# index-tts/index-tts

Measured on AMD Instinct MI355X. Metric: audio-seconds/sec (RTF) IndexTTS-2.5, 64-utt batch @1/2/4/8 MI355X, higher is better.
Workload: dtype bf16 (GPT GEMM operands / KV cache; f32 accumulate, residual stream, norms: the reference's own GPU mode) + fp32x3 (flow matching: f32 activations / weights / accumulation, GEMM and attention products on the bf16 matrix pipe with every f32 operand carried exactly as three bf16 planes = 24 significan

## Files before the change

include/indextts_hip.h:

```cpp
#ifndef INDEXTTS_HIP_H
#define INDEXTTS_HIP_H

#include <stddef.h>
#include <stdint.h>

#ifdef __cplusplus
extern "C" {
#endif

#define ITTS_ABI_VERSION 13

int itts_abi_version(void);
const char* itts_last_error(void);
int itts_device_count(void);

int itts_set_option(const char* name, int value);
int itts_get_option(const char* name, int* value);
int itts_reset_options(void);
int itts_option_count(void);
const char* itts_option_name(int index);
const char* itts_option_doc(int index);
int itts_option_default(int index);


// ... 108 lines not shown
void itts_gpt_destroy(itts_gpt* h);
size_t itts_gpt_workspace_bytes(const itts_gpt* h, int nseq, int S, int Tmax);

int itts_gpt_generate(itts_gpt* h, const float* prefix_embeds, const int32_t* pad_lens, int nseq, int S,
                      const itts_gen_params* params, const int32_t* penalty_ids, int n_penalty_ids,
                      const double* uniforms, int64_t* codes_out, int32_t* n_steps_out, void* workspace,
                      size_t workspace_bytes, int use_graph, void* stream);
int itts_gpt_generate_chunk(itts_gpt* h, const float* prefix_embeds, const int32_t* pad_lens, int nseq, int S,
                            const itts_gen_params* params, const int32_t* penalty_ids, int n_penalty_ids,
                            const double* uniforms, int64_t* codes_out, int32_t step_limit, int32_t* n_steps_out,
                            void* workspace, size_t workspace_bytes, int use_graph, void* stream);
size_t itts_gpt_admit_workspace_bytes(const itts_gpt* h, int n_new, int S_new);
int itts_gpt_admit_rows(itts_gpt* h, const float* prefix_embeds, const int32_t* pad_lens, const int32_t* slots, int n_new, int S_new,
                        const int32_t* row_limits_new, const itts_gen_params* params, const int32_t* penalty_ids, int n_penalty_ids,
                        const double* uniforms, int64_t* codes_out, void* workspace, size_t workspace_bytes, void* admit_workspace,
                        size_t admit_bytes, void* stream);
size_t itts_gpt_beam_workspace_bytes(const itts_gpt* h, int n_utts, int num_beams, int S, int Tmax);
int itts_gpt_generate_beam(itts_gpt* h, const float* prefix_embeds, const int32_t* pad_lens, int n_utts, int num_beams,
                           int S, const itts_gen_params* params, const int32_t* penalty_ids, int n_penalty_ids,
                           const double* uniforms, int32_t* hist_tok_out, int32_t* hist_par_out, float* beam_scores_out,
                           float* hyps_out, int32_t* n_hyps_out, uint8_t* done_out, int32_t* n_steps_out,
                           void* workspace, size_t workspace_bytes, int use_graph, void* stream);
int itts_gpt_generate_beam_chunk(itts_gpt* h, const float* prefix_embeds, const int32_t* pad_lens, int n_utts, int num_beams, int S,
                                 const itts_gen_params* params, const int32_t* penalty_ids, int n_penalty_ids, const int32_t* group_caps,
                                 int32_t* hist_tok_out, int32_t* hist_par_out, float* beam_scores_out, float* hyps_out, int32_t* n_hyps_out,
                                 uint8_t* done_out, int32_t step_limit, int32_t* n_steps_out, void* workspace, size_t workspace_bytes,
                                 int use_graph, void* stream);
size_t itts_gpt_admit_beam_workspace_bytes(const itts_gpt* h, int n_new, int S_new);
int itts_gpt_admit_beam_groups(itts_gpt* h, const float* prefix_embeds, const int32_t* pad_lens, const int32_t* slots, int n_new, int S_new,
                               const int32_t* group_caps_new, const itts_gen_params* params, const int32_t* penalty_ids, int n_penalty_ids,
                               void* workspace, size_t workspace_bytes, void* admit_workspace, size_t admit_bytes, void* stream);
int itts_gpt_last_timing(const itts_gpt* h, float* prefill_ms, float* decode_ms, int32_t* steps);
int itts_gpt_graph_stats(const itts_gpt* h, int32_t* captures, int32_t* hits);
int itts_gpt_set_compaction(itts_gpt* h, int enable, int granularity);
int itts_gpt_set_chunk_return(itts_gpt* h, int finished_rows);
int itts_gpt_set_row_limits(itts_gpt* h, const int32_t* limits, int n);
typedef struct {
    int32_t  do_sample, top_k, min_tokens_to_keep;
    float    top_p, temperature, repetition_penalty, typical_mass;
    int32_t  stream;
    uint64_t seed;
} itts_row_sampling;
int itts_gpt_set_row_sampling(itts_gpt* h, const itts_row_sampling* table, int n);
typedef struct {
    int32_t  do_sample, top_k, min_tokens_to_keep;
    float    top_p, temperature, repetition_penalty, typical_mass, length_penalty;
    int32_t  stream;
    uint64_t seed;
} itts_group_sampling;
int itts_gpt_set_group_sampling(itts_gpt* h, const itts_group_sampling* table, int n_groups);
typedef struct {
    int32_t  min_new_tokens;
    int32_t  min_length;
    int32_t  no_repeat_ngram_size;
    int32_t  decay_start;
    float    min_p;
    float    epsilon_cutoff;
    float    eta_cutoff;
    int32_t  n_suppress, n_begin_suppress, n_decay;
    const int32_t* suppress_ids;
    const int32_t* begin_suppress_ids;
    const float*   decay_table;
} itts_logits_filters;
int itts_gpt_set_logits_filters(itts_gpt* h, const itts_logits_filters* f);
int itts_gpt_compaction_stats(const itts_gpt* h, int64_t* row_steps, int32_t* compactions);

int itts_gpt_forward_latent(itts_gpt* h, const float* x, int nseq, int S, float* out, void* workspace,
                            size_t workspace_bytes, void* stream);

typedef struct itts_gpt_latent itts_gpt_latent;
size_t itts_gpt_latent_workspace_bytes(const itts_gpt* h, int nseq, int max_prefix, int max_codes, int max_append);
int itts_gpt_latent_open(itts_gpt* h, const float* prefix_x, const int32_t* prefix_lens, int nseq, int max_prefix, int max_codes,
                         int max_append, void* workspace, size_t workspace_bytes, void* stream, itts_gpt_latent** session);
int itts_gpt_latent_append(itts_gpt_latent* session, const int64_t* codes, int n, float* out, void* stream);
int itts_gpt_latent_appended(const itts_gpt_latent* session);
int itts_gpt_latent_close(itts_gpt_latent* session);

int itts_gemm_tile_occupancy(int precision, int32_t* blocks_per_cu);
const char* itts_gemm_last_path(void);
int itts_gemm_path_count(void);
const char* itts_gemm_path_name(int index);
int itts_gemm_forward(const void* A, const void* Wp, const float* bias, float* out, int M, int N, int K, int precision,
                      int prefill_tiles, int gelu, void* stream);
int itts_layernorm_forward(const float* x, const float* gamma, const float* beta, const float* gamma2,
                           const float* beta2, float* out, int rows, int D, float eps, void* stream);
const char* itts_attention_last_path(void);
int itts_attention_path_count(void);
const char* itts_attention_path_name(int index);
int itts_gpt_attention_forward(const float* q, const void* kcache, const void* vcache, void* out, const int32_t* pos_ptr, const int32_t* pad,
                               const int32_t* pos_shift, const int32_t* seq_map, const int32_t* row_map, const int32_t* row_map_alt,
                               const int32_t* step_ptr, int nseq, int heads, int nq, int Tmax, int seq_mul, int precision, void* stream);
int itts_gemm_ln_forward(const float* x, const float* partial, const float* bias_prev, const float* ln_gamma, const float* ln_beta, float eps,
                         const void* Wp, const float* bias, float* out, float* x_out, int M, int N, int K, void* stream);

typedef struct {
    int32_t hidden_dim, num_heads, depth;
    int32_t in_channels;
    int32_t wavenet_hidden, wavenet_layers, wavenet_kernel, wavenet_dilation_rate;
    int32_t precision;
    float norm_eps;
} itts_s2mel_config;

typedef struct itts_s2mel itts_s2mel;

int itts_s2mel_create(const itts_s2mel_config* cfg, itts_s2mel** out);
int itts_s2mel_device(const itts_s2mel* h);
int itts_s2mel_load_tensor(itts_s2mel* h, const char* name, const float* host_data, const int64_t* shape, int ndim);
int itts_s2mel_finalize(itts_s2mel* h);
void itts_s2mel_destroy(itts_s2mel* h);
size_t itts_s2mel_workspace_bytes(const itts_s2mel* h, int n_tok, int n_seq, int t_max);
int itts_s2mel_mods_per_step(const itts_s2mel* h);

int itts_s2mel_estimator(itts_s2mel* h, const float* x, const float* const_in, const float* mods, const float* rope,
                         const int32_t* tok_seq, const int32_t* tok_t, const int32_t* seq_start, const int32_t* seq_T,
                         const int32_t* seq_len, int n_seq, int n_tok, int t_max, float* d_out, void* workspace,
                         size_t workspace_bytes, void* stream);
int itts_s2mel_solve(itts_s2mel* h, float* x_state, const float* const_in, const float* mods, const float* rope,
                     const int32_t* tok_seq, const int32_t* tok_t, const int32_t* seq_start, const int32_t* seq_T,
                     const int32_t* seq_len, const int32_t* prompt_len, int n_seq, int n_tok, int t_max, int n_branch, int n_steps,
                     const float* t_span, float cfg_rate, void* workspace, size_t workspace_bytes, void* stream);

int itts_s2mel_set_profiling(itts_s2mel* h, int enable);
int itts_s2mel_profile_read(itts_s2mel* h, double* ms, double* launches, double* flops);

int itts_s2mel_set_trace(itts_s2mel* h, void* dev_u64, int capacity);
int itts_s2mel_trace_count(const itts_s2mel* h);
int itts_s2mel_trace_wanted(const itts_s2mel* h);
const char* itts_s2mel_trace_label(const itts_s2mel* h, int index);
int itts_s2mel_set_capture(itts_s2mel* h, void* dev_buf, size_t bytes, const char* label_prefix);
long long itts_s2mel_capture_offset(const itts_s2mel* h, int index, size_t* bytes);

int itts_s2mel_set_tail(itts_s2mel* h, const int32_t* tok_seq, const int32_t* tok_t, const int32_t* seq_start, const int32_t* seq_T,
                        const int32_t* seq_len, const int32_t* tail_src, const int32_t* tail_base, int n_seq, int n_tail, int t_max);

int itts_s2mel_noise_forward(float* x_rows, const int32_t* tok_seq, const int32_t* tok_t, const int32_t* prompt_len,
                             const uint64_t* seq_seed, const uint64_t* seq_key, const float* seq_temperature,
                             int n_seq, int n_rows, int channels, void* stream);

size_t itts_s2mel_attention_scratch_bytes(int n_tok, int n_seq, int heads, int t_max, int precision);
int itts_s2mel_attention_forward(const float* qkv, const float* rope, const int32_t* tok_seq, const int32_t* tok_t,
                                 const int32_t* seq_start, const int32_t* seq_T, const int32_t* seq_len, int n_seq, int n_tok,
                                 int t_max, int heads, int precision, void* out, void* scratch, size_t scratch_bytes, void* stream);

int itts_vq_project_forward(const int64_t* codes, const float* codebook, const float* w, const float* bias, float* out, int n,
                            int n_codes, int cd, int H, void* stream);
int itts_vq_search_forward(const float* h, const float* w_in, const float* b_in, const float* cb_norm, const float* cb_sq, int64_t* idx,
                           int n, int H, int n_codes, int cd, void* stream);
int itts_tok_gather_conv_forward(const float* x, float* col, const int32_t* tok_seq, const int32_t* tok_t, const int32_t* src_start,
                                 const int32_t* src_T, const int32_t* dst_T, int n_dst, int C, int k, void* stream);
int itts_tok_dwconv_forward(const float* x, const float* w, const float* b, float* y, const int32_t* tok_seq, const int32_t* tok_t,
                            const int32_t* seq_T, int n, int C, int k, void* stream);
int itts_tok_gelu_forward(float* x, size_t n, void* stream);
int itts_tok_scale_residual_forward(float* x, const float* y, const float* gamma, int n, int C, void* stream);
int itts_tok_groupnorm_mish_forward(float* x, const float* gamma, const float* beta, const int32_t* seq_start, const int32_t* seq_T,
                                    int n_seq, int C, float eps, void* stream);

int itts_attention_forward(const float* q, const float* k, const float* v, float* out, const int32_t* kstart, const int32_t* klen,
                           int n_q, int heads, int dq, int dv, float scale, void* stream);
int itts_attention_relkey_forward(const float* q, const float* k, const float* v, float* out, const int32_t* kstart, const int32_t* klen,
                                  const int32_t* qpos, const float* dist_emb, int left, int right, int n_q, int heads, int dq, int dv,
                                  float scale, void* stream);
int itts_tok_dwconv_causal_forward(const float* x, const float* w, const float* b, float* y, const int32_t* tok_seq, const int32_t* tok_t,
                                   const int32_t* seq_T, int n, int C, int k, void* stream);
int itts_tok_glu_forward(const float* x, float* out, int n, int C, int mode, void* stream);
int itts_tok_act_forward(float* x, size_t n, int mode, void* stream);
int itts_tok_l2norm_forward(float* x, const float* gamma, int n, int C, float scale, void* stream);
// ... 35 lines not shown
```

indextts_amd/_lib.py:

```python
import ctypes as C
import os

HERE = os.path.dirname(os.path.abspath(__file__))
LIB_PATH = os.path.join(HERE, "csrc", "libindextts_hip.so")

c_f32p = C.POINTER(C.c_float)
c_i32p = C.POINTER(C.c_int32)
c_i64p = C.POINTER(C.c_int64)
vp = C.c_void_p


class BigVGANConfig(C.Structure):
    _fields_ = [
        ("in_channels", C.c_int32), ("upsample_initial_channel", C.c_int32), ("num_upsamples", C.c_int32),
        ("upsample_rates", C.c_int32 * 8), ("upsample_kernel_sizes", C.c_int32 * 8), ("num_kernels", C.c_int32),
        ("resblock_kernel_sizes", C.c_int32 * 4), ("num_dilations", C.c_int32),
        ("resblock_dilations", (C.c_int32 * 4) * 4), ("snake_logscale", C.c_int32), ("activation", C.c_int32),
        ("use_tanh_at_final", C.c_int32), ("use_bias_at_final", C.c_int32), ("cond_dim", C.c_int32),
        ("cond_in_each_up_layer", C.c_int32),
    ]


class S2MelConfig(C.Structure):
    _fields_ = [("hidden_dim", C.c_int32), ("num_heads", C.c_int32), ("depth", C.c_int32), ("in_channels", C.c_int32),
# ... 92 lines not shown
    "itts_packed_gemm_bytes": (C.c_size_t, [C.c_int, C.c_int, C.c_int]),
    "itts_pack_gemm_weight": (C.c_int, [vp, C.c_int, C.c_int, C.c_int, C.c_int, vp]),
    "itts_gpt_create": (C.c_int, [C.POINTER(GPTConfig), C.POINTER(vp)]),
    "itts_gpt_device": (C.c_int, [vp]),
    "itts_gpt_load_tensor": (C.c_int, [vp, C.c_char_p, vp, c_i64p, C.c_int]),
    "itts_gpt_finalize": (C.c_int, [vp]),
    "itts_gpt_destroy": (None, [vp]),
    "itts_gpt_workspace_bytes": (C.c_size_t, [vp, C.c_int, C.c_int, C.c_int]),
    "itts_gpt_generate": (C.c_int, [vp, vp, vp, C.c_int, C.c_int, C.POINTER(GenParams), c_i32p, C.c_int, vp, vp,
                                    C.POINTER(C.c_int32), vp, C.c_size_t, C.c_int, vp]),
    "itts_gpt_generate_chunk": (C.c_int, [vp, vp, vp, C.c_int, C.c_int, C.POINTER(GenParams), c_i32p, C.c_int, vp, vp, C.c_int32,
                                          C.POINTER(C.c_int32), vp, C.c_size_t, C.c_int, vp]),
    "itts_gpt_beam_workspace_bytes": (C.c_size_t, [vp, C.c_int, C.c_int, C.c_int, C.c_int]),
    "itts_gpt_generate_beam": (C.c_int, [vp, vp, vp, C.c_int, C.c_int, C.c_int, C.POINTER(GenParams), c_i32p, C.c_int, vp,
                                         vp, vp, vp, vp, vp, vp, C.POINTER(C.c_int32), vp, C.c_size_t, C.c_int, vp]),
    "itts_gpt_admit_workspace_bytes": (C.c_size_t, [vp, C.c_int, C.c_int]),
    "itts_gpt_admit_rows": (C.c_int, [vp, vp, vp, vp, C.c_int, C.c_int, vp, vp, vp, C.c_int, vp, vp, vp, C.c_size_t, vp, C.c_size_t, vp]),
    "itts_gpt_generate_beam_chunk": (C.c_int, [vp, vp, vp, C.c_int, C.c_int, C.c_int, C.POINTER(GenParams), c_i32p, C.c_int, c_i32p,
                                               vp, vp, vp, vp, vp, vp, C.c_int32, C.POINTER(C.c_int32), vp, C.c_size_t, C.c_int, vp]),
    "itts_gpt_admit_beam_workspace_bytes": (C.c_size_t, [vp, C.c_int, C.c_int]),
    "itts_gpt_admit_beam_groups": (C.c_int, [vp, vp, vp, c_i32p, C.c_int, C.c_int, c_i32p, C.POINTER(GenParams), c_i32p, C.c_int,
                                             vp, C.c_size_t, vp, C.c_size_t, vp]),
    "itts_gpt_last_timing": (C.c_int, [vp, C.POINTER(C.c_float), C.POINTER(C.c_float), C.POINTER(C.c_int32)]),
    "itts_gpt_graph_stats": (C.c_int, [vp, C.POINTER(C.c_int32), C.POINTER(C.c_int32)]),
    "itts_gpt_set_compaction": (C.c_int, [vp, C.c_int, C.c_int]),
    "itts_gpt_set_row_limits": (C.c_int, [vp, vp, C.c_int]),
    "itts_gpt_set_row_sampling": (C.c_int, [vp, vp, C.c_int]),
    "itts_gpt_set_group_sampling": (C.c_int, [vp, vp, C.c_int]),
    "itts_gpt_set_logits_filters": (C.c_int, [vp, C.POINTER(LogitsFilters)]),
    "itts_gpt_set_chunk_return": (C.c_int, [vp, C.c_int]),
    "itts_gpt_compaction_stats": (C.c_int, [vp, C.POINTER(C.c_int64), C.POINTER(C.c_int32)]),
    "itts_gpt_forward_latent": (C.c_int, [vp, vp, C.c_int, C.c_int, vp, vp, C.c_size_t, vp]),
    "itts_gpt_latent_workspace_bytes": (C.c_size_t, [vp, C.c_int, C.c_int, C.c_int, C.c_int]),
    "itts_gpt_latent_open": (C.c_int, [vp, vp, c_i32p, C.c_int, C.c_int, C.c_int, C.c_int, vp, C.c_size_t, vp, C.POINTER(vp)]),
    "itts_gpt_latent_append": (C.c_int, [vp, vp, C.c_int, vp, vp]),
    "itts_gpt_latent_appended": (C.c_int, [vp]),
    "itts_gpt_latent_close": (C.c_int, [vp]),
    "itts_gemm_tile_occupancy": (C.c_int, [C.c_int, C.POINTER(C.c_int32)]),
    "itts_s2mel_create": (C.c_int, [C.POINTER(S2MelConfig), C.POINTER(vp)]),
    "itts_s2mel_device": (C.c_int, [vp]),
    "itts_s2mel_load_tensor": (C.c_int, [vp, C.c_char_p, vp, c_i64p, C.c_int]),
    "itts_s2mel_set_tail": (C.c_int, [vp, vp, vp, vp, vp, vp, vp, vp, C.c_int, C.c_int, C.c_int]),
    "itts_s2mel_finalize": (C.c_int, [vp]),
    "itts_s2mel_destroy": (None, [vp]),
    "itts_s2mel_workspace_bytes": (C.c_size_t, [vp, C.c_int, C.c_int, C.c_int]),
    "itts_s2mel_mods_per_step": (C.c_int, [vp]),
    "itts_s2mel_estimator": (C.c_int, [vp, vp, vp, vp, vp, vp, vp, vp, vp, vp, C.c_int, C.c_int, C.c_int, vp, vp, C.c_size_t, vp]),
    "itts_s2mel_solve": (C.c_int, [vp, vp, vp, vp, vp, vp, vp, vp, vp, vp, vp, C.c_int, C.c_int, C.c_int, C.c_int, C.c_int,
                                   C.POINTER(C.c_float), C.c_float, vp, C.c_size_t, vp]),
    "itts_s2mel_set_profiling": (C.c_int, [vp, C.c_int]),
    "itts_s2mel_profile_read": (C.c_int, [vp, vp, vp, vp]),
    "itts_s2mel_set_trace": (C.c_int, [vp, vp, C.c_int]),
    "itts_s2mel_trace_count": (C.c_int, [vp]),
    "itts_s2mel_trace_wanted": (C.c_int, [vp]),
    "itts_s2mel_trace_label": (C.c_char_p, [vp, C.c_int]),
    "itts_s2mel_set_capture": (C.c_int, [vp, vp, C.c_size_t, C.c_char_p]),
    "itts_s2mel_capture_offset": (C.c_longlong, [vp, C.c_int, C.POINTER(C.c_size_t)]),
    "itts_s2mel_noise_forward": (C.c_int, [vp, vp, vp, vp, vp, vp, vp, C.c_int, C.c_int, C.c_int, vp]),
    "itts_s2mel_attention_scratch_bytes": (C.c_size_t, [C.c_int, C.c_int, C.c_int, C.c_int, C.c_int]),
    "itts_s2mel_attention_forward": (C.c_int, [vp, vp, vp, vp, vp, vp, vp, C.c_int, C.c_int, C.c_int, C.c_int, C.c_int, vp, vp,
                                               C.c_size_t, vp]),
    "itts_vq_project_forward": (C.c_int, [vp, vp, vp, vp, vp, C.c_int, C.c_int, C.c_int, C.c_int, vp]),
    "itts_vq_search_forward": (C.c_int, [vp, vp, vp, vp, vp, vp, C.c_int, C.c_int, C.c_int, C.c_int, vp]),
    "itts_tok_gather_conv_forward": (C.c_int, [vp, vp, vp, vp, vp, vp, vp, C.c_int, C.c_int, C.c_int, vp]),
    "itts_tok_dwconv_forward": (C.c_int, [vp, vp, vp, vp, vp, vp, vp, C.c_int, C.c_int, C.c_int, vp]),
    "itts_tok_gelu_forward": (C.c_int, [vp, C.c_size_t, vp]),
    "itts_attention_forward": (C.c_int, [vp, vp, vp, vp, vp, vp, C.c_int, C.c_int, C.c_int, C.c_int, C.c_float, vp]),
    "itts_attention_relkey_forward": (C.c_int, [vp, vp, vp, vp, vp, vp, vp, vp, C.c_int, C.c_int, C.c_int, C.c_int, C.c_int, C.c_int, C.c_float, vp]),
    "itts_tok_dwconv_causal_forward": (C.c_int, [vp, vp, vp, vp, vp, vp, vp, C.c_int, C.c_int, C.c_int, vp]),
    "itts_tok_glu_forward": (C.c_int, [vp, vp, C.c_int, C.c_int, C.c_int, vp]),
    "itts_tok_act_forward": (C.c_int, [vp, C.c_size_t, C.c_int, vp]),
    "itts_tok_l2norm_forward": (C.c_int, [vp, vp, C.c_int, C.c_int, C.c_float, vp]),
    "itts_tok_affine_forward": (C.c_int, [vp, C.c_int, vp, vp, vp, C.c_int, C.c_int, C.c_int, vp]),
    "itts_tok_ctxpool_forward": (C.c_int, [vp, vp, C.c_int, C.c_int, C.c_int, vp]),
    "itts_tok_gate_forward": (C.c_int, [vp, vp, C.c_size_t, vp]),
    "itts_tok_attnstats_forward": (C.c_int, [vp, vp, vp, C.c_int, C.c_int, C.c_float, vp]),
    "itts_tok_statspool_forward": (C.c_int, [vp, vp, C.c_int, C.c_int, vp]),
    "itts_tok_scale_residual_forward": (C.c_int, [vp, vp, vp, C.c_int, C.c_int, vp]),
    "itts_tok_groupnorm_mish_forward": (C.c_int, [vp, vp, vp, vp, vp, C.c_int, C.c_int, C.c_float, vp]),
    "itts_gemm_last_path": (C.c_char_p, []),
    "itts_gemm_path_count": (C.c_int, []),
    "itts_gemm_path_name": (C.c_char_p, [C.c_int]),
    "itts_gemm_forward": (C.c_int, [vp, vp, vp, vp, C.c_int, C.c_int, C.c_int, C.c_int, C.c_int, C.c_int, vp]),
    "itts_attention_last_path": (C.c_char_p, []),
    "itts_attention_path_count": (C.c_int, []),
    "itts_attention_path_name": (C.c_char_p, [C.c_int]),
    "itts_gpt_attention_forward": (C.c_int, [vp, vp, vp, vp, vp, vp, vp, vp, vp, vp, vp, C.c_int, C.c_int, C.c_int, C.c_int, C.c_int, C.c_int, vp]),
    "itts_layernorm_forward": (C.c_int, [vp, vp, vp, vp, vp, vp, C.c_int, C.c_int, C.c_float, vp]),
    "itts_gemm_ln_forward": (C.c_int, [vp, vp, vp, vp, vp, C.c_float, vp, vp, vp, vp, C.c_int, C.c_int, C.c_int, vp]),
    "itts_fbank_frames": (C.c_int, [C.POINTER(FbankConfig), C.c_int]),
    "itts_fbank_forward": (C.c_int, [vp, C.c_int, C.c_int, C.c_int64, C.POINTER(FbankConfig), vp, vp, vp, vp, C.c_int, C.c_int64, vp]),
    "itts_resample_forward": (C.c_int, [vp, vp, vp, C.c_int, C.c_int, C.c_int64, C.c_int, C.c_int64, C.c_int, C.c_int, C.c_int, vp]),
    "itts_tok_colnorm_forward": (C.c_int, [vp, vp, C.c_int, C.c_int, C.c_int, C.c_int, C.c_int, C.c_float, vp]),
}

_lib = None


class HipEngineError(RuntimeError):
    pass


def lib():
    global _lib
    if _lib is None:
        if not os.path.exists(LIB_PATH):
            raise HipEngineError(
                f"{LIB_PATH} is missing: build it with `python indextts_amd/build.py` (hipcc, gfx950). "
                "The engine has no CPU fallback.")
        import torch
        L = C.CDLL(LIB_PATH)
        for name, (res, args) in SIGNATURES.items():
            fn = getattr(L, name)
            fn.restype = res
            fn.argtypes = args
        if L.itts_abi_version() != ABI_VERSION:
            raise HipEngineError("libindextts_hip.so ABI version mismatch")
        _lib = L
    return _lib


def check(rc: int, what: str = ""):
    if rc != 0:
        msg = lib().itts_last_error().decode(errors="replace")
        raise HipEngineError(f"{what} failed (code {rc}): {msg}")


def set_option(name: str, value: int):
    check(lib().itts_set_option(name.encode(), int(value)), f"set_option({name})")


def get_option(name: str) -> int:
    v = C.c_int(0)
    check(lib().itts_get_option(name.encode(), C.byref(v)), f"get_option({name})")
    return int(v.value)


def reset_options():
    check(lib().itts_reset_options(), "reset_options")


def options() -> dict:
    L = lib()
    out = {}
    for i in range(L.itts_option_count()):
        name = L.itts_option_name(i).decode()
        out[name] = (get_option(name), int(L.itts_option_default(i)), L.itts_option_doc(i).decode())
    return out


def gemm_last_path() -> str:
    return lib().itts_gemm_last_path().decode()


def gemm_path_names() -> list:
    L = lib()
    return [L.itts_gemm_path_name(i).decode() for i in range(L.itts_gemm_path_count())]


def attention_last_path() -> str:
    return lib().itts_attention_last_path().decode()


def attention_path_names() -> list:
    L = lib()
    return [L.itts_attention_path_name(i).decode() for i in range(L.itts_attention_path_count())]
# ... 39 lines not shown
```

indextts_amd/csrc/capi_gpt.hip:

```cpp
#include <math.h>
#include <stddef.h>
#include <string.h>
#include <mutex>
#include <set>
#include <string>
#include <vector>

#include "../../include/indextts_hip.h"
#include "gpt_kernels.h"

extern "C" size_t itts_packed_gemm_bytes(int K, int N, int precision) {
    if (precision == PREC_F32X3) return (size_t)((N + 15) / 16) * (K / 32) * 3 * 64 * 16;
    const int KB = precision == PREC_BF16 ? 32 : 16;
    return (size_t)((N + 15) / 16) * (K / KB) * 64 * 16;
}

extern "C" int itts_pack_gemm_weight(const float* w, int K, int N, int transposed, int precision, void* out) {
    const int KB = precision == PREC_F32 ? 16 : 32;
    if (!w || !out || K <= 0 || N <= 0 || K % KB) {
        itts_set_error("pack_gemm: K=%d must be a positive multiple of %d", K, KB);
        return ITTS_ERR_ARG;
    }
    if (precision != PREC_F32 && precision != PREC_BF16 && precision != PREC_F32X3) { itts_set_error("pack_gemm: precision %d", precision); return ITTS_ERR_ARG; }
    const int ntiles = (N + 15) / 16, nkb = K / KB, per = KB / 4;
// ... 1608 lines not shown
    s->base = base; s->shift = shift_dev; s->last = last_dev;
    { std::lock_guard<std::mutex> lk(g_latent_mu); g_latent_live.insert(s); }
    *out = s;
    return ITTS_OK;
}

extern "C" int itts_gpt_latent_append(itts_gpt_latent* s, const int64_t* codes, int n, float* out, void* caller_stream) {
    if (!s || !codes || !out) { itts_set_error("gpt_latent_append: null pointer"); return ITTS_ERR_ARG; }
    {
        std::lock_guard<std::mutex> lk(g_latent_mu);
        if (!g_latent_live.count(s)) { itts_set_error("gpt_latent_append: the session is closed"); return ITTS_ERR_STATE; }
    }
    itts_gpt* h = s->h;
    const itts_gpt_config& c = h->cfg;
    if (n < 1 || n > s->max_append) { itts_set_error("gpt_latent_append: n = %d outside 1 .. max_append = %d", n, s->max_append); return ITTS_ERR_ARG; }
    if (s->appended + n > s->max_codes) {
        itts_set_error("gpt_latent_append: %d + %d codes exceed the session's max_codes = %d", s->appended, n, s->max_codes);
        return ITTS_ERR_ARG;
    }
    if (s->appended + n > c.n_mel_pos) {
        itts_set_error("gpt_latent_append: mel position %d is past the mel position table (%d rows)", s->appended + n - 1, c.n_mel_pos);
        return ITTS_ERR_ARG;
    }
    ItDevGuard dg(h->device);
    if (int rcd = check_same_device(h, codes, out, "gpt_latent_append")) return rcd;
    const GptWs w = carve(c, s->base, s->nseq, s->Smax, s->Tmax);
    hipStream_t st = h->stream, cs = (hipStream_t)caller_stream;
    if (int rcs = stream_enter(h, cs)) return rcs;
    hipLaunchKernelGGL(set_state_kernel, dim3(1), dim3(1), 0, st, w.state, 0, s->max_prefix + s->appended);
    hipLaunchKernelGGL(latent_embed_kernel, dim3(n, s->nseq), dim3(256), 0, st, (const long long*)codes, n, s->last + (size_t)s->parity * s->nseq,
                       s->last + (size_t)(s->parity ^ 1) * s->nseq, s->appended, c.start_mel_token, c.vocab, h->mel_emb, h->mel_pos, w.x, c.model_dim);
    HIP_TRY(hipGetLastError());
    bool pending = false;
    int rc = run_layers(h, w, s->nseq, n, s->Tmax, true, w.state + 1, nullptr, &pending, st, false, 1, nullptr, nullptr, s->shift);
    if (rc) return rc;
    LnArgs ln{};
    ln.x = w.x; ln.g1 = h->lnf_g; ln.b1 = h->lnf_b; ln.g2 = h->fn_g; ln.b2 = h->fn_b; ln.out = out; ln.out_f32 = 1;
    ln.rows = s->nseq * n; ln.D = c.model_dim; ln.in_row_mul = 1; ln.in_row_add = 0; ln.eps = c.ln_eps; ln.nsplit = 1;
    if ((rc = launch_ln(ln, c.precision, st))) return rc;
    if ((rc = stream_leave(h, cs))) return rc;
    s->appended += n;
    s->parity ^= 1;
    return ITTS_OK;
}

extern "C" int itts_gpt_latent_appended(const itts_gpt_latent* s) {
    std::lock_guard<std::mutex> lk(g_latent_mu);
    return (s && g_latent_live.count(const_cast<itts_gpt_latent*>(s))) ? s->appended : -1;
}

extern "C" int itts_gpt_latent_close(itts_gpt_latent* s) {
    if (!s) { itts_set_error("gpt_latent_close: null"); return ITTS_ERR_ARG; }
    std::lock_guard<std::mutex> lk(g_latent_mu);
    if (!g_latent_live.erase(s)) { itts_set_error("gpt_latent_close: the session is already closed"); return ITTS_ERR_STATE; }
    delete s;
    return ITTS_OK;
}

extern "C" int itts_gemm_tile_occupancy(int precision, int32_t* blocks_per_cu) {
    if (!blocks_per_cu) { itts_set_error("gemm_tile_occupancy: null"); return ITTS_ERR_ARG; }
    int n = 0;
    const int rc = gemm_tile_occupancy(precision, &n);
    *blocks_per_cu = n;
    return rc;
}

extern "C" const char* itts_gemm_last_path(void) {
    const char* n = gemm_path_name(gemm_last_path());
    return n ? n : "none";
}
extern "C" int itts_gemm_path_count(void) { return GP_COUNT; }
extern "C" const char* itts_gemm_path_name(int index) { return gemm_path_name(index); }

extern "C" int itts_gemm_forward(const void* A, const void* Wp, const float* bias, float* out, int M, int N, int K,
                                 int precision, int prefill_tiles, int gelu, void* stream) {
    if (!A || !Wp || !out) { itts_set_error("gemm_forward: null pointer"); return ITTS_ERR_ARG; }
    GemmArgs g{};
    g.A = A; g.lda = K; g.Wp = Wp; g.bias = bias; g.M = M; g.N = N; g.K = K; g.nsplit = 1; g.D = N;
    g.epi = EPI_STORE_F32; g.out_f32 = out; g.ldo = N;
    (void)gelu;
    return launch_gemm(g, precision, prefill_tiles != 0, (hipStream_t)stream);
}

extern "C" const char* itts_attention_last_path(void) {
    const char* n = attention_path_name(attention_last_path());
    return n ? n : "none";
}
extern "C" int itts_attention_path_count(void) { return AP_COUNT; }
extern "C" const char* itts_attention_path_name(int index) { return attention_path_name(index); }

extern "C" int itts_gpt_attention_forward(const float* q, const void* kcache, const void* vcache, void* out, const int32_t* pos_ptr,
                                          const int32_t* pad, const int32_t* pos_shift, const int32_t* seq_map, const int32_t* row_map,
                                          const int32_t* row_map_alt, const int32_t* step_ptr, int nseq, int heads, int nq, int Tmax, int seq_mul,
                                          int precision, void* stream) {
    if (!q || !kcache || !vcache || !out || !pos_ptr) { itts_set_error("gpt_attention_forward: null pointer"); return ITTS_ERR_ARG; }
    if (precision != PREC_F32 && precision != PREC_BF16) {
        itts_set_error("gpt_attention_forward: precision %d (0 f32 or 1 bf16; the KV-cache attention has no fp32x3 form)", precision);
        return ITTS_ERR_ARG;
    }
    if (nseq < 1 || heads < 1 || nq < 1 || nq > 65535 || Tmax < 1 || seq_mul < 0) {
        itts_set_error("gpt_attention_forward: nseq=%d heads=%d nq=%d (1..65535) Tmax=%d seq_mul=%d out of range", nseq, heads, nq, Tmax, seq_mul);
        return ITTS_ERR_ARG;
    }
    if ((long long)nseq * heads > 0x7fffffffLL) { itts_set_error("gpt_attention_forward: nseq * heads = %lld blocks", (long long)nseq * heads); return ITTS_ERR_ARG; }
    if ((row_map_alt || step_ptr) && !(row_map && row_map_alt && step_ptr)) {
        itts_set_error("gpt_attention_forward: row_map_alt and step_ptr come together, and with a row_map");
        return ITTS_ERR_ARG;
    }
    AttnArgs at{};
    at.qbuf = q; at.kcache = kcache; at.vcache = vcache; at.pad = pad; at.pos_ptr = pos_ptr; at.pos_shift = pos_shift;
    at.row_map = row_map; at.row_map_alt = row_map_alt; at.step_ptr = step_ptr;
    at.out = out; at.nseq = nseq; at.H = heads; at.nq = nq; at.Tmax = Tmax; at.D = heads * 64; at.seq_mul = seq_mul; at.seq_map = seq_map;
    return launch_attention(at, precision, (hipStream_t)stream);
}

extern "C" int itts_gemm_ln_forward(const float* x, const float* partial, const float* bias_prev, const float* ln_gamma, const float* ln_beta,
                                    float eps, const void* Wp, const float* bias, float* out, float* x_out, int M, int N, int K, void* stream) {
    if (!x || !ln_gamma || !ln_beta || !Wp || !out) { itts_set_error("gemm_ln_forward: null pointer"); return ITTS_ERR_ARG; }
    if (!gemm_decode_ln_ok(M, K, EPI_STORE_F32)) { itts_set_error("gemm_ln_forward: M = %d (1..16), K = %d (256, 512, 1280) unsupported", M, K); return ITTS_ERR_ARG; }
    GemmArgs g{};
    g.Wp = Wp; g.bias = bias; g.M = M; g.N = N; g.K = K; g.nsplit = 1; g.D = N;
    g.epi = EPI_STORE_F32; g.out_f32 = out; g.ldo = N;
    g.ln_x = x; g.ln_partial = partial; g.ln_bias_prev = bias_prev; g.ln_g = ln_gamma; g.ln_b = ln_beta; g.ln_eps = eps; g.ln_x_out = x_out;
    return launch_gemm_decode_ln(g, (hipStream_t)stream);
}

extern "C" int itts_layernorm_forward(const float* x, const float* gamma, const float* beta, const float* gamma2,
                                      const float* beta2, float* out, int rows, int D, float eps, void* stream) {
    if (!x || !gamma || !beta || !out) { itts_set_error("layernorm_forward: null pointer"); return ITTS_ERR_ARG; }
    LnArgs ln{};
    ln.x = const_cast<float*>(x); ln.g1 = gamma; ln.b1 = beta; ln.g2 = gamma2; ln.b2 = beta2; ln.out = out; ln.out_f32 = 1;
    ln.rows = rows; ln.D = D; ln.in_row_mul = 1; ln.in_row_add = 0; ln.eps = eps; ln.nsplit = 1;
    return launch_ln(ln, PREC_F32, (hipStream_t)stream);
}
```

indextts_amd/csrc/capi_s2mel.hip:

```cpp
#include <math.h>
#include <stdlib.h>
#include <string.h>
#include <algorithm>
#include <map>
#include <string>
#include <vector>

#include "../../include/indextts_hip.h"
#include "gpt_kernels.h"
#include "s2mel_kernels.h"

static bool s2_fused(int precision, bool opt_fused) {
    if (precision == PREC_F32X3) return true;
    return (precision == PREC_BF16 || precision == PREC_F32) && opt_fused;
}

struct S2Layer {
    void *w_qkv = 0, *w_o = 0, *w_13 = 0, *w_2 = 0, *w_skip_a = 0, *w_skip_b = 0;
    float *g_attn = 0, *g_ffn = 0, *b_skip = 0;
};
struct S2Wn {
    void *w_in = 0, *w_rs = 0;
    float *b_in = 0, *b_rs = 0;
};

struct itts_s2mel {
    itts_s2mel_config cfg;
    int I = 0, Kx = 0;
    std::map<std::string, std::pair<std::vector<float>, std::vector<int64_t>>> host;
    std::vector<S2Layer> layers;
    std::vector<S2Wn> wn;
    float* g_norm = 0;
    void *w_x = 0, *w_sl_a = 0, *w_sl_b = 0, *w_c1 = 0, *w_rp = 0, *w_fl = 0, *w_c2 = 0;
    float *b_sl = 0, *b_c1 = 0, *b_rp = 0, *b_fl = 0, *b_c2 = 0;
    std::vector<void*> owned;
    bool finalized = false;
    bool opt_fused = true;
    bool opt_fused_qkv = true;
    int device = -1;
    bool profiling = false;
    std::vector<hipEvent_t> ev_pool;
    struct Rec { int cls; double flops; };
    std::vector<Rec> recs;
    hipStream_t prof_stream = nullptr;
    SeqTab tail{};
    const int* tail_src = nullptr;
    const int* tail_base = nullptr;
    bool tail_set = false;
    unsigned long long* trace = nullptr;
    int trace_cap = 0, trace_n = 0;
    int trace_wanted = 0;
    std::vector<const char*> trace_labels;
    char* capture = nullptr;
    size_t capture_bytes = 0, capture_used = 0;
    std::string capture_prefix;
    std::vector<long long> capture_off;
    std::vector<size_t> capture_len;
};

static int s2_trace(itts_s2mel* h, hipStream_t st, const char* label, const void* p, size_t bytes) {
    if (!h->trace) return ITTS_OK;
    ++h->trace_wanted;
    if (h->trace_n >= h->trace_cap) return ITTS_OK;
    if ((int)h->trace_labels.size() <= h->trace_n) { h->trace_labels.push_back(label); h->capture_off.push_back(-1); h->capture_len.push_back(0); }
    else { h->trace_labels[h->trace_n] = label; h->capture_off[h->trace_n] = -1; h->capture_len[h->trace_n] = 0; }
    if (h->capture && !h->capture_prefix.empty() && strncmp(label, h->capture_prefix.c_str(), h->capture_prefix.size()) == 0) {
        const size_t at = (h->capture_used + 255) & ~(size_t)255;
        if (at + bytes <= h->capture_bytes) {
            HIP_TRY(hipMemcpyAsync(h->capture + at, p, bytes, hipMemcpyDeviceToDevice, st));
            h->capture_off[h->trace_n] = (long long)at;
            h->capture_len[h->trace_n] = bytes;
            h->capture_used = at + bytes;
        }
    }
    return launch_trace_hash(p, bytes, h->trace + h->trace_n++, st);
}
static int s2_trace_begin(itts_s2mel* h, hipStream_t st) {
    h->trace_n = 0;
    h->trace_wanted = 0;
    h->capture_used = 0;
    if (h->trace && h->trace_cap > 0) HIP_TRY(hipMemsetAsync(h->trace, 0, (size_t)h->trace_cap * 8, st));
    return ITTS_OK;
}

enum { S2_GEMM = 0, S2_ATTN = 1, S2_OTHER = 2, S2_CLASSES = 3 };

struct S2Prof {
    itts_s2mel* h;
    hipStream_t st;
    bool on;
    size_t idx;
    S2Prof(itts_s2mel* h_, hipStream_t st_, int cls, double flops) : h(h_), st(st_), on(h_->profiling), idx(0) {
        if (!on) return;
        idx = h->recs.size();
        h->recs.push_back({cls, flops});
        while (h->ev_pool.size() < 2 * (idx + 1)) {
            hipEvent_t e;
            if (hipEventCreate(&e) != hipSuccess) { on = false; h->recs.pop_back(); return; }
// ... 210 lines not shown
    NEED(wc2, P + "conv2.weight", C, W);
    NEED(bc2, P + "conv2.bias", C);
    if (rc == ITTS_OK && gn && wmerge && wsl && bsl && wc1 && bc1 && wrp && brp && wfl && bfl && wc2 && bc2) {
        const int ldm = (int)h->host[P + "cond_x_merge_linear.weight"].second.back();
        if (ldm < C) { itts_set_error("s2mel_finalize: cond_x_merge_linear has %d input columns, fewer than the mel channels", ldm); return ITTS_ERR_ARG; }
        rc = f.vec(gn, &h->g_norm);
        if (!rc) rc = f.pack_kn(Fin::cols_kn(*wmerge, H, ldm, 0, C), C, Kx, H, &h->w_x);
        if (!rc) rc = f.pack_kn(Fin::cols_kn(*wsl, H, H + C, 0, H), H, H, H, &h->w_sl_a);
        if (!rc) rc = f.pack_kn(Fin::cols_kn(*wsl, H, H + C, H, C), C, Kx, H, &h->w_sl_b);
        if (!rc) rc = f.vec(bsl, &h->b_sl);
        if (!rc) rc = f.pack_kn(Fin::cols_kn(*wc1, W, H, 0, H), H, H, W, &h->w_c1);
        if (!rc) rc = f.vec(bc1, &h->b_c1);
        if (!rc) rc = f.pack_kn(Fin::cols_kn(*wrp, W, H, 0, H), H, H, W, &h->w_rp);
        if (!rc) rc = f.vec(brp, &h->b_rp);
        if (!rc) rc = f.pack_kn(Fin::cols_kn(*wfl, W, W, 0, W), W, W, W, &h->w_fl);
        if (!rc) rc = f.vec(bfl, &h->b_fl);
        if (!rc) rc = f.pack_kn(Fin::cols_kn(*wc2, C, W, 0, W), W, W, C, &h->w_c2);
        if (!rc) rc = f.vec(bc2, &h->b_c2);
    }
    for (int i = 0; i < L && rc == ITTS_OK; ++i) {
        const std::string a = P + "wavenet.in_layers." + std::to_string(i) + ".conv.conv.", b = P + "wavenet.res_skip_layers." + std::to_string(i) + ".conv.conv.";
        const int ro = i < L - 1 ? 2 * W : W;
        NEED(wi, a + "weight", 2 * W, W, k);
        NEED(bi, a + "bias", 2 * W);
        NEED(wr, b + "weight", ro, W, 1);
        NEED(br, b + "bias", ro);
        if (!wi || !bi || !wr || !br) continue;
        std::vector<float> kn((size_t)k * W * 2 * W);
        for (int n = 0; n < 2 * W; ++n)
            for (int cc = 0; cc < W; ++cc)
                for (int j = 0; j < k; ++j) kn[((size_t)j * W + cc) * 2 * W + n] = (*wi)[((size_t)n * W + cc) * k + j];
        rc = f.pack_kn(f.pair_tiles(kn, k * W, 2 * W), k * W, k * W, 2 * W, &h->wn[i].w_in);
        if (!rc) rc = f.vec(bi, &h->wn[i].b_in);
        if (!rc) rc = f.pack_kn(Fin::cols_kn(*wr, ro, W, 0, W), W, W, ro, &h->wn[i].w_rs);
        if (!rc) rc = f.vec(br, &h->wn[i].b_rs);
    }
#undef NEED
    if (rc) return rc;
    if (!f.missing.empty()) { itts_set_error("s2mel_finalize: missing or mis-shaped tensors: %s", f.missing.c_str()); return ITTS_ERR_STATE; }
    h->host.clear();
    h->finalized = true;
    return ITTS_OK;
}

extern "C" int itts_s2mel_mods_per_step(const itts_s2mel* h) {
    if (!h) return 0;
    const itts_s2mel_config& c = h->cfg;
    return c.depth * 4 * c.hidden_dim + 2 * c.hidden_dim + c.wavenet_layers * 2 * c.wavenet_hidden + 2 * c.wavenet_hidden;
}

static size_t s_a256(size_t x) { return (x + 255) & ~(size_t)255; }

struct S2Ws {
    float *X, *X2, *BIG, *WX, *OUT, *RP, *D;
    char *HB, *QA, *AO, *FC, *COL, *XA, *SK, *KC, *VC, *WXA, *ZR, *HBP;
    size_t hbp_stride;
    size_t sk_stride, total;
};

static S2Ws s2_carve(const itts_s2mel* h, char* base, int n_tok, int n_seq, int t_pad) {
    const itts_s2mel_config& c = h->cfg;
    const size_t N = (size_t)n_tok, H = c.hidden_dim, I = h->I, W = c.wavenet_hidden, C = c.in_channels, Kx = h->Kx;
    const size_t esz = c.precision == PREC_BF16 ? 2 : 4;
    const size_t big = std::max(std::max(3 * H, 2 * I), 2 * W);
    const size_t hw = std::max(H, W), fw = std::max(I, W);
    S2Ws w;
    size_t off = 0;
    auto take = [&](size_t bytes) { char* p = base ? base + off : nullptr; off += s_a256(bytes); return p; };
    w.X = (float*)take(N * H * 4);
    w.X2 = (float*)take(N * H * 4);
    w.BIG = (float*)take(N * big * 4);
    w.WX = (float*)take(N * W * 4);
    w.OUT = (float*)take(N * W * 4);
    w.RP = (float*)take(N * W * 4);
    w.D = (float*)take(N * C * 4);
    w.HB = take(N * hw * esz);
    w.QA = take(N * H * esz);
    w.AO = take(N * H * esz);
    w.FC = take(N * fw * esz);
    w.COL = take(N * (size_t)c.wavenet_kernel * W * esz);
    w.XA = take(N * Kx * esz);
    w.sk_stride = s_a256(N * H * esz);
    w.SK = take(w.sk_stride * (size_t)(c.depth / 2));
    w.WXA = take(N * W * esz);
    w.hbp_stride = (N * H + 127) / 128 * 128;
    w.HBP = take(c.precision == PREC_F32X3 ? w.hbp_stride * 6 : 0);
    const size_t kv = (size_t)n_seq * c.num_heads * t_pad * 64 * (c.precision == PREC_F32X3 ? 6 : esz);
    w.ZR = take(256);
    w.KC = take(kv);
    w.VC = take(kv);
    w.total = off + 256;
    return w;
}

extern "C" size_t itts_s2mel_workspace_bytes(const itts_s2mel* h, int n_tok, int n_seq, int t_max) {
    if (!h || n_tok <= 0 || n_seq <= 0 || t_max <= 0) return 0;
    return s2_carve(h, nullptr, n_tok, n_seq, (t_max + 63) / 64 * 64).total;
}

static int s2_launch_gemm(itts_s2mel* h, const GemmArgs& g, hipStream_t st) {
    S2Prof ps(h, st, S2_GEMM, 2.0 * g.M * (double)g.N * g.K);
    return launch_gemm(g, h->cfg.precision, true, st);
}

static int s2_gemm(itts_s2mel* h, const void* A, int lda, const void* Wp, const float* bias, float* out, int ldo, int M, int N, int K,
                   int epi, hipStream_t st, void* shadow = nullptr) {
    GemmArgs g{};
    g.A = A; g.lda = lda; g.Wp = Wp; g.bias = bias; g.M = M; g.N = N; g.K = K; g.nsplit = 1; g.epi = epi; g.out_f32 = out; g.ldo = ldo; g.D = N;
    g.out_act2 = shadow;
    return s2_launch_gemm(h, g, st);
}

static int s2_estimator(itts_s2mel* h, const S2Ws& w, const SeqTab& tab, int t_pad, const float* x_src, int src_rows, const float* const_in,
                        const float* mods, const float* rope, float* d_out, hipStream_t st, double attn_flops = 0.0,
                        const SeqTab* tail = nullptr, const int* tail_src = nullptr) {
    S2Prof whole(h, st, S2_OTHER, 0.0);
    const itts_s2mel_config& c = h->cfg;
    const int H = c.hidden_dim, I = h->I, W = c.wavenet_hidden, C = c.in_channels, Kx = h->Kx, N = tab.n_tok, prec = c.precision;
    const int nh = c.num_heads;
    const bool fused = s2_fused(prec, h->opt_fused);
    const bool x3_attn = prec == PREC_F32X3 && itts_opt(OPT_X3_ATTN) != 0;
    const size_t kv_plane = (size_t)tab.n_seq * nh * t_pad * 64;
    const bool a_planes = prec == PREC_F32X3 && fused && itts_opt(OPT_X3_APLANES) != 0 && itts_opt(OPT_X3_PRODUCTS) == 6 && itts_opt(OPT_X3_SCHED) != 0 && H % 32 == 0;
    const bool prune_opt = prec == PREC_F32X3 && fused && itts_opt(OPT_S2MEL_PRUNE_LAST) != 0;
    const bool prune_last = prune_opt && x3_attn && tail != nullptr && c.depth > 0;
    int rc;
    float *X = w.X, *X2 = w.X2;
    const size_t esz = prec == PREC_BF16 ? 2 : 4;
    const size_t kvb = kv_plane * (prec == PREC_F32X3 ? (x3_attn ? 6 : 4) : esz);
#define S2_TRACE(label, ptr, bytes) do { if (h->trace && (rc = s2_trace(h, st, label, ptr, bytes))) return rc; } while (0)
    if ((rc = launch_cast_pad(x_src, w.XA, N, src_rows, C, Kx, prec, st))) return rc;
    if (!prune_opt) HIP_TRY(hipMemcpyAsync(X, const_in, (size_t)N * H * 4, hipMemcpyDeviceToDevice, st));
    S2_TRACE("cast_pad(x) -> XA", w.XA, (size_t)N * Kx * esz);
    if (prune_opt) {
        GemmArgs g{};
        g.A = w.XA; g.lda = Kx; g.Wp = h->w_x; g.M = N; g.N = H; g.K = Kx; g.nsplit = 1; g.epi = EPI_RESIDUAL_SRC; g.out_f32 = X; g.ldo = H; g.D = H;
        g.res_src = const_in;
        if ((rc = s2_launch_gemm(h, g, st))) return rc;
    } else if ((rc = s2_gemm(h, w.XA, Kx, h->w_x, nullptr, X, H, N, H, Kx, EPI_RESIDUAL, st))) return rc;
    S2_TRACE("x_in GEMM -> X", X, (size_t)N * H * 4);
    int n_skip = 0;
    for (int i = 0; i < c.depth; ++i) {
        const S2Layer& L = h->layers[i];
        if (i > c.depth / 2) {
            if (!fused && (rc = launch_cast_pad(X, w.HB, N, N, H, H, prec, st))) return rc;
            --n_skip;
            if ((rc = s2_gemm(h, w.HB, H, L.w_skip_a, L.b_skip, X2, H, N, H, H, EPI_STORE_F32, st))) return rc;
            if ((rc = s2_gemm(h, w.SK + w.sk_stride * n_skip, H, L.w_skip_b, nullptr, X2, H, N, H, H, EPI_RESIDUAL, st))) return rc;
            S2_TRACE("skip_in GEMMs -> X", X2, (size_t)N * H * 4);
            float* tmp = X; X = X2; X2 = tmp;
        }
        if (a_planes) {
            if ((rc = launch_ada_rmsnorm_planes(X, L.g_attn, mods + (size_t)i * 4 * H, w.HBP, w.hbp_stride, N, H, c.norm_eps, st))) return rc;
            S2_TRACE("ada_rmsnorm(attn) -> HB planes", w.HBP, w.hbp_stride * 6);
        } else {
            if ((rc = launch_ada_rmsnorm(X, L.g_attn, mods + (size_t)i * 4 * H, w.HB, N, H, c.norm_eps, prec, st))) return rc;
            S2_TRACE("ada_rmsnorm(attn) -> HB", w.HB, (size_t)N * H * esz);
        }
        if (fused && h->opt_fused_qkv) {
            GemmArgs g{};
            g.A = w.HB; g.lda = H; g.Wp = L.w_qkv; g.M = N; g.N = 3 * H; g.K = H; g.nsplit = 1; g.epi = EPI_QKV_ROPE;
            if (a_planes) { g.A = w.HBP; g.a_planes = w.hbp_stride; }
            g.out_act = w.QA; g.kcache = w.KC; g.vcache = w.VC; g.D = H; g.H = nh; g.Tmax = t_pad;
            g.tok_seq = tab.tok_seq; g.tok_t = tab.tok_t; g.rope = rope;
            g.kv_planes = x3_attn ? kv_plane : 0;
            if ((rc = s2_launch_gemm(h, g, st))) return rc;
        } else {
            if ((rc = s2_gemm(h, w.HB, H, L.w_qkv, nullptr, w.BIG, 3 * H, N, 3 * H, H, EPI_STORE_F32, st))) return rc;
            if ((rc = launch_rope_split(w.BIG, rope, w.QA, w.KC, w.VC, tab, nh, t_pad, prec, st))) return rc;
        }
        S2_TRACE("wqkv -> Q", w.QA, (size_t)N * H * esz);
        S2_TRACE("wqkv -> K", w.KC, kvb);
        S2_TRACE("wqkv -> V^T", w.VC, kvb);
        const bool pruned = prune_last && i == c.depth - 1;
        const int NL = pruned ? tail->n_tok : N;
        { S2Prof ps(h, st, S2_ATTN, attn_flops * ((double)NL / (double)N));
          if (x3_attn) rc = launch_s2mel_attention_x3(w.QA, w.KC, w.VC, w.AO, tab, nh, t_pad, st, pruned ? tail : nullptr);
          else rc = launch_s2mel_attention(w.QA, w.KC, w.VC, w.AO, tab, nh, t_pad, prec, st);
          if (rc) return rc; }
        S2_TRACE("attention -> AO", w.AO, (size_t)NL * H * esz);
        if (pruned) {
            GemmArgs g{};
            g.A = w.AO; g.lda = H; g.Wp = L.w_o; g.M = NL; g.N = H; g.K = H; g.nsplit = 1; g.epi = EPI_RESIDUAL_SRC; g.out_f32 = X2; g.ldo = H; g.D = H;
            g.res_src = X; g.res_map = tail_src;
            if ((rc = s2_launch_gemm(h, g, st))) return rc;
            float* tmp = X; X = X2; X2 = tmp;
        } else if ((rc = s2_gemm(h, w.AO, H, L.w_o, nullptr, X, H, N, H, H, EPI_RESIDUAL, st))) return rc;
        S2_TRACE("wo GEMM -> X", X, (size_t)NL * H * 4);
        if (a_planes) {
            if ((rc = launch_ada_rmsnorm_planes(X, L.g_ffn, mods + (size_t)i * 4 * H + 2 * H, w.HBP, w.hbp_stride, NL, H, c.norm_eps, st))) return rc;
            S2_TRACE("ada_rmsnorm(ffn) -> HB planes", w.HBP, w.hbp_stride * 6);
        } else {
            if ((rc = launch_ada_rmsnorm(X, L.g_ffn, mods + (size_t)i * 4 * H + 2 * H, w.HB, NL, H, c.norm_eps, prec, st))) return rc;
            S2_TRACE("ada_rmsnorm(ffn) -> HB", w.HB, (size_t)NL * H * esz);
        }
        if (fused) {
            GemmArgs g{};
            g.A = w.HB; g.lda = H; g.Wp = L.w_13; g.M = NL; g.N = 2 * I; g.K = H; g.nsplit = 1; g.epi = EPI_SWIGLU; g.out_act = w.FC; g.D = I;
            if (a_planes) { g.A = w.HBP; g.a_planes = w.hbp_stride; }
            if ((rc = s2_launch_gemm(h, g, st))) return rc;
        } else {
            if ((rc = s2_gemm(h, w.HB, H, L.w_13, nullptr, w.BIG, 2 * I, NL, 2 * I, H, EPI_STORE_F32, st))) return rc;
            if ((rc = launch_swiglu(w.BIG, w.FC, NL, I, prec, st))) return rc;
        }
        void* shadow = nullptr;
        if (fused && i < c.depth / 2) shadow = w.SK + w.sk_stride * n_skip;
        else if (fused && i + 1 < c.depth && i + 1 > c.depth / 2) shadow = w.HB;
        S2_TRACE("w13 + SwiGLU -> FC", w.FC, (size_t)NL * I * esz);
        if ((rc = s2_gemm(h, w.FC, I, L.w_2, nullptr, X, H, NL, H, I, EPI_RESIDUAL, st, shadow))) return rc;
        S2_TRACE("w2 GEMM -> X", X, (size_t)NL * H * 4);
        if (i < c.depth / 2) {
            if (!fused && (rc = launch_cast_pad(X, w.SK + w.sk_stride * n_skip, N, N, H, H, prec, st))) return rc;
            ++n_skip;
        }
    }
    const float* m_norm = mods + (size_t)c.depth * 4 * H;
    const float* m_gc = m_norm + 2 * H;
    const float* m_fl = m_gc + (size_t)c.wavenet_layers * 2 * W;
    const SeqTab& tt = tail ? *tail : tab;
    const void* XAt = w.XA;
    if (tail) {
        if ((rc = launch_cast_pad(x_src, w.QA, tail->n_tok, src_rows, C, Kx, prec, st, tail_src))) return rc;
        XAt = w.QA;
    }
    const int NT = tt.n_tok;
    if ((rc = launch_ada_rmsnorm(X, h->g_norm, m_norm, w.HB, NT, H, c.norm_eps, prec, st, tail && !prune_last ? tail_src : nullptr))) return rc;
    S2_TRACE("final ada_rmsnorm -> HB", w.HB, (size_t)NT * H * esz);
    if ((rc = s2_gemm(h, w.HB, H, h->w_sl_a, h->b_sl, X2, H, NT, H, H, EPI_STORE_F32, st))) return rc;
    if ((rc = s2_gemm(h, XAt, Kx, h->w_sl_b, nullptr, X2, H, NT, H, Kx, EPI_RESIDUAL, st, fused ? w.HB : nullptr))) return rc;
    if (!fused && (rc = launch_cast_pad(X2, w.HB, NT, NT, H, H, prec, st))) return rc;
    S2_TRACE("skip_linear -> X2", X2, (size_t)NT * H * 4);
    if ((rc = s2_gemm(h, w.HB, H, h->w_c1, h->b_c1, w.WX, W, NT, W, H, EPI_STORE_F32, st, fused ? w.WXA : nullptr))) return rc;
    S2_TRACE("conv1 -> WX", w.WX, (size_t)NT * W * 4);
    if ((rc = s2_gemm(h, w.HB, H, h->w_rp, h->b_rp, w.RP, W, NT, W, H, EPI_STORE_F32, st))) return rc;
    int dil = 1;
    for (int i = 0; i < c.wavenet_layers; ++i) {
        const S2Wn& Wn = h->wn[i];
        const int last = i == c.wavenet_layers - 1;
        if (!fused && (rc = launch_im2col_reflect(w.WX, w.COL, tt, W, c.wavenet_kernel, dil, prec, st))) return rc;
        const int ro = last ? W : 2 * W;
        if (fused) {
            GemmArgs g{};
            g.A = w.WXA; g.lda = W; g.Wp = Wn.w_in; g.bias = Wn.b_in; g.M = NT; g.N = 2 * W; g.K = c.wavenet_kernel * W;
            g.nsplit = 1; g.epi = EPI_GATE; g.out_act = w.FC; g.gvec = m_gc + (size_t)i * 2 * W; g.D = W;
            g.conv_taps = c.wavenet_kernel; g.conv_dil = dil; g.conv_W = W; g.tok_seq = tt.tok_seq; g.tok_t = tt.tok_t;
            g.seq_start = tt.seq_start; g.seq_T = tt.seq_T; g.zero_row = w.ZR;
            if ((rc = s2_launch_gemm(h, g, st))) return rc;
            GemmArgs r{};
            r.A = w.FC; r.lda = W; r.Wp = Wn.w_rs; r.bias = Wn.b_rs; r.M = NT; r.N = ro; r.K = W; r.nsplit = 1; r.epi = EPI_WN_RS;
            r.out_f32 = w.WX; r.out2 = w.OUT; r.D = W; r.wn_first = i == 0; r.wn_last = last; r.out_act2 = last ? nullptr : w.WXA;
            r.tok_seq = tt.tok_seq; r.tok_t = tt.tok_t; r.seq_len = tt.seq_len;
            S2_TRACE("wavenet in_layer + gate -> FC", w.FC, (size_t)NT * W * esz);
            if ((rc = s2_launch_gemm(h, r, st))) return rc;
            S2_TRACE("wavenet res_skip -> WX", w.WX, (size_t)NT * W * 4);
            S2_TRACE("wavenet res_skip -> OUT", w.OUT, (size_t)NT * W * 4);
        } else {
            if ((rc = s2_gemm(h, w.COL, c.wavenet_kernel * W, Wn.w_in, Wn.b_in, w.BIG, 2 * W, NT, 2 * W, c.wavenet_kernel * W, EPI_STORE_F32, st))) return rc;
            if ((rc = launch_wn_gate(w.BIG, m_gc + (size_t)i * 2 * W, w.FC, NT, W, prec, st))) return rc;
            if ((rc = s2_gemm(h, w.FC, W, Wn.w_rs, Wn.b_rs, w.BIG, ro, NT, ro, W, EPI_STORE_F32, st))) return rc;
            if ((rc = launch_wn_update(w.BIG, w.WX, w.OUT, tt, W, i == 0, last, st))) return rc;
        }
        dil *= c.wavenet_dilation_rate;
    }
    if ((rc = launch_final_ln_mod(w.OUT, w.RP, m_fl, w.HB, tt, W, prec, st))) return rc;
    if ((rc = s2_gemm(h, w.HB, W, h->w_fl, h->b_fl, w.BIG, W, NT, W, W, EPI_STORE_F32, st, fused ? w.FC : nullptr))) return rc;
    if (!fused && (rc = launch_cast_pad(w.BIG, w.FC, NT, NT, W, W, prec, st))) return rc;
    S2_TRACE("final_layer -> FC", w.FC, (size_t)NT * W * esz);
    if ((rc = s2_gemm(h, w.FC, W, h->w_c2, h->b_c2, d_out, C, NT, C, W, EPI_STORE_F32, st))) return rc;
    S2_TRACE("conv2 -> output", d_out, (size_t)NT * C * 4);
    return ITTS_OK;
#undef S2_TRACE
}

static int s2_check(const itts_s2mel* h, const void* a, const void* b, const char* who) {
    const int da = itts_ptr_device(a), db = itts_ptr_device(b);
    if ((da >= 0 && da != h->device) || (db >= 0 && db != h->device)) {
        itts_set_error("%s: tensors are on device %d/%d but the model was created on device %d", who, da, db, h->device);
        return ITTS_ERR_ARG;
    }
    return ITTS_OK;
}

static SeqTab s2_tab(const int32_t* tok_seq, const int32_t* tok_t, const int32_t* seq_start, const int32_t* seq_T, const int32_t* seq_len,
                     int n_seq, int n_tok, int t_max) {
    SeqTab t;
    t.tok_seq = tok_seq; t.tok_t = tok_t; t.seq_start = seq_start; t.seq_T = seq_T; t.seq_len = seq_len;
    t.n_seq = n_seq; t.n_tok = n_tok; t.t_max = t_max;
    return t;
}

extern "C" int itts_s2mel_estimator(itts_s2mel* h, const float* x, const float* const_in, const float* mods, const float* rope,
                                    const int32_t* tok_seq, const int32_t* tok_t, const int32_t* seq_start, const int32_t* seq_T,
                                    const int32_t* seq_len, int n_seq, int n_tok, int t_max, float* d_out, void* workspace,
                                    size_t workspace_bytes, void* stream) {
    if (!h || !x || !const_in || !mods || !rope || !tok_seq || !tok_t || !seq_start || !seq_T || !seq_len || !d_out || !workspace) {
        itts_set_error("s2mel_estimator: null pointer");
        return ITTS_ERR_ARG;
    }
    if (!h->finalized) { itts_set_error("s2mel_estimator: call itts_s2mel_finalize first"); return ITTS_ERR_STATE; }
    if (n_seq <= 0 || n_tok <= 0 || t_max <= 0) { itts_set_error("s2mel_estimator: bad sizes"); return ITTS_ERR_ARG; }
    ItDevGuard dg(h->device);
    if (int rc = s2_check(h, x, workspace, "s2mel_estimator")) return rc;
    const int t_pad = (t_max + 63) / 64 * 64;
    const S2Ws w0 = s2_carve(h, nullptr, n_tok, n_seq, t_pad);
    if (workspace_bytes < w0.total) { itts_set_error("s2mel_estimator: workspace too small (%zu < %zu)", workspace_bytes, w0.total); return ITTS_ERR_ARG; }
    char* base = (char*)(((uintptr_t)workspace + 255) & ~(uintptr_t)255);
    const S2Ws w = s2_carve(h, base, n_tok, n_seq, t_pad);
    hipStream_t st = (hipStream_t)stream;
    const size_t kv = (size_t)((char*)w.VC - (char*)w.KC);
    HIP_TRY(hipMemsetAsync(w.ZR, 0, (size_t)((char*)w.KC - (char*)w.ZR) + 2 * kv, st));
    const SeqTab tab = s2_tab(tok_seq, tok_t, seq_start, seq_T, seq_len, n_seq, n_tok, t_max);
    h->recs.clear();
    h->prof_stream = st;
    if (int rc = s2_trace_begin(h, st)) return rc;
    return s2_estimator(h, w, tab, t_pad, x, n_tok, const_in, mods, rope, d_out, st);
}

extern "C" int itts_s2mel_solve(itts_s2mel* h, float* x_state, const float* const_in, const float* mods, const float* rope,
                                const int32_t* tok_seq, const int32_t* tok_t, const int32_t* seq_start, const int32_t* seq_T,
                                const int32_t* seq_len, const int32_t* prompt_len, int n_seq, int n_tok, int t_max, int n_branch,
                                int n_steps, const float* t_span, float cfg_rate, void* workspace, size_t workspace_bytes, void* stream) {
    if (!h || !x_state || !const_in || !mods || !rope || !tok_seq || !tok_t || !seq_start || !seq_T || !seq_len || !prompt_len || !t_span || !workspace) {
        itts_set_error("s2mel_solve: null pointer");
        return ITTS_ERR_ARG;
    }
    if (!h->finalized) { itts_set_error("s2mel_solve: call itts_s2mel_finalize first"); return ITTS_ERR_STATE; }
    if (n_seq <= 0 || n_tok <= 0 || t_max <= 0 || n_steps < 1 || (n_branch != 1 && n_branch != 2) || n_tok % n_branch || n_seq % n_branch) {
        itts_set_error("s2mel_solve: bad sizes (n_seq=%d n_tok=%d n_branch=%d n_steps=%d)", n_seq, n_tok, n_branch, n_steps);
        return ITTS_ERR_ARG;
    }
    ItDevGuard dg(h->device);
    if (int rc = s2_check(h, x_state, workspace, "s2mel_solve")) return rc;
    const int t_pad = (t_max + 63) / 64 * 64;
    const S2Ws w0 = s2_carve(h, nullptr, n_tok, n_seq, t_pad);
    if (workspace_bytes < w0.total) { itts_set_error("s2mel_solve: workspace too small (%zu < %zu)", workspace_bytes, w0.total); return ITTS_ERR_ARG; }
    char* base = (char*)(((uintptr_t)workspace + 255) & ~(uintptr_t)255);
    const S2Ws w = s2_carve(h, base, n_tok, n_seq, t_pad);
    hipStream_t st = (hipStream_t)stream;
    const size_t kv = (size_t)((char*)w.VC - (char*)w.KC);
    HIP_TRY(hipMemsetAsync(w.ZR, 0, (size_t)((char*)w.KC - (char*)w.ZR) + 2 * kv, st));
    const SeqTab tab = s2_tab(tok_seq, tok_t, seq_start, seq_T, seq_len, n_seq, n_tok, t_max);
    const int mps = itts_s2mel_mods_per_step(h);
    h->recs.clear();
    h->prof_stream = st;
    if (int rc = s2_trace_begin(h, st)) return rc;
    for (int step = 0; step < n_steps; ++step) {
        const bool use_tail = h->tail_set && h->tail.n_seq == n_seq && h->tail.n_tok > 0 && h->tail.n_tok <= n_tok && h->tail.n_tok % n_branch == 0;
        int rc = s2_estimator(h, w, tab, t_pad, x_state, n_tok / n_branch, const_in, mods + (size_t)step * mps, rope, w.D, st, 0.0,
                              use_tail ? &h->tail : nullptr, use_tail ? h->tail_src : nullptr);
        if (rc) return rc;
        const float dt = t_span[step + 1] - t_span[step];
// ... 77 lines not shown
```

indextts_amd/csrc/common.h:

```cpp
#pragma once
#include <hip/hip_runtime.h>
#include <stdint.h>
#include <stdio.h>
#include <string.h>

#define ITTS_OK 0
#define ITTS_ERR_ARG 1
#define ITTS_ERR_HIP 2
#define ITTS_ERR_STATE 3
#define ITTS_ERR_NOMEM 4

#define HIP_TRY(expr)                                                                         \
    do {                                                                                      \
        hipError_t _e = (expr);                                                               \
        if (_e != hipSuccess) {                                                               \
            itts_set_error("%s:%d %s -> %s", __FILE__, __LINE__, #expr, hipGetErrorString(_e)); \
            return ITTS_ERR_HIP;                                                              \
        }                                                                                     \
    } while (0)

void itts_set_error(const char* fmt, ...);

enum { OPT_DECODE_FUSE_LN, OPT_DECODE_GEMM, OPT_DECODE_ROT, OPT_DECODE_WNT, OPT_DECODE_NT, OPT_PREFILL_GEMM, OPT_TILE256, OPT_F32_TILE,
       OPT_X3_PRODUCTS, OPT_X3_SCHED, OPT_X3_ATTN, OPT_SAMPLE_RADIX, OPT_GPT_COMPACT, OPT_ATTN_WAVES, OPT_S2MEL_FUSED, OPT_FA_QS,
       OPT_F32_ATTN_SCALAR, OPT_FA32_QS, OPT_AA_ACT, OPT_CONV_BM, OPT_H3_KERNEL, OPT_DECODE_LN_NT, OPT_X3_APLANES, OPT_X3_PIN, OPT_PREFILL_ATTN, OPT_VOC_ACT_PLANES, OPT_X3_WAVES, OPT_S2MEL_PRUNE_LAST, OPT_X3_ATTN_SKIP, OPT_COUNT };
int itts_opt(int id);
unsigned itts_opt_epoch();

typedef float f32x4 __attribute__((ext_vector_type(4)));
typedef float f32x16 __attribute__((ext_vector_type(16)));
typedef short bf16x8 __attribute__((ext_vector_type(8)));
typedef unsigned short u16;

static inline int ceil_div(int a, int b) { return (a + b - 1) / b; }

struct ItDevGuard {
    int prev = -1;
    bool switched = false;
    explicit ItDevGuard(int dev) {
        if (dev < 0) return;
        if (hipGetDevice(&prev) != hipSuccess) { prev = -1; (void)hipGetLastError(); }
        if (prev != dev && hipSetDevice(dev) == hipSuccess) switched = true;
    }
    ~ItDevGuard() { if (switched && prev >= 0) (void)hipSetDevice(prev); }
    ItDevGuard(const ItDevGuard&) = delete;
    ItDevGuard& operator=(const ItDevGuard&) = delete;
};
static inline int itts_current_device() {
    int d = -1;
    if (hipGetDevice(&d) != hipSuccess) { d = -1; (void)hipGetLastError(); }
    return d;
}
static inline int itts_ptr_device(const void* p) {
    hipPointerAttribute_t at;
    if (!p || hipPointerGetAttributes(&at, p) != hipSuccess) { (void)hipGetLastError(); return -1; }
    return at.type == hipMemoryTypeDevice ? at.device : -1;
}

template <class T>
struct ItPerDevice {
    T v[32] = {};
    T& cur() {
        const int d = itts_current_device();
        return v[(d >= 0 && d < 32) ? d : 0];
    }
};

#ifdef __HIPCC__
__device__ __forceinline__ float wave_sum(float v) {
#pragma unroll
    for (int o = 32; o > 0; o >>= 1) v += __shfl_xor(v, o, 64);
    return v;
}
__device__ __forceinline__ float wave_max(float v) {
#pragma unroll
    for (int o = 32; o > 0; o >>= 1) v = fmaxf(v, __shfl_xor(v, o, 64));
    return v;
}
__device__ __forceinline__ float bf16_to_f32(u16 h) { return __uint_as_float(((uint32_t)h) << 16); }
__device__ __forceinline__ u16 f32_to_bf16(float f) {
    uint32_t u = __float_as_uint(f);
    if ((u & 0x7fffffffu) > 0x7f800000u) return (u16)((u >> 16) | 0x40);
    u += 0x7fffu + ((u >> 16) & 1u);
    return (u16)(u >> 16);
}
#endif

static inline u16 host_f32_to_bf16(float f) {
    uint32_t u;
    memcpy(&u, &f, 4);
    if ((u & 0x7fffffffu) > 0x7f800000u) return (u16)((u >> 16) | 0x40);
    u += 0x7fffu + ((u >> 16) & 1u);
    return (u16)(u >> 16);
}
```

indextts_amd/csrc/gemm_tile.h:

```cpp
#pragma once
#include "gpt_kernels.h"
#include <type_traits>

typedef __bf16 bf16x8_t __attribute__((ext_vector_type(8)));
typedef unsigned int v4u __attribute__((ext_vector_type(4)));

__device__ __forceinline__ float gelu_new_f(float x) {
    const float c = 0.7978845608028654f;
    return 0.5f * x * (1.0f + tanhf(c * (x + 0.044715f * x * x * x)));
}

#define PF_BM 128
#define PF_BN 128
#define PF_BK 64
#define PF_GM 8
#define PF_LDS 67584
#ifndef PF_SCHED
#define PF_SCHED 1
#endif

__device__ __forceinline__ uint32_t pf_pack2(float a, float b) { return (uint32_t)f32_to_bf16(a) | ((uint32_t)f32_to_bf16(b) << 16); }

template <int EPI>
__device__ __forceinline__ void pf_epilogue(const GemmArgs& a, int mbase, int nbase, int lane, f32x4 v) {
// ... 259 lines not shown
                    vt[0] = (u16)(pk.x & 0xffffu);
                    vt[(size_t)a.Tmax] = (u16)(pk.x >> 16);
                    vt[(size_t)2 * a.Tmax] = (u16)(pk.y & 0xffffu);
                    vt[(size_t)3 * a.Tmax] = (u16)(pk.y >> 16);
                }
            }
        }
    }
}

template <int ROWS, int NT, bool F32 = false>
__device__ __forceinline__ void pf_store_vt(const GemmArgs& a, const float* ctT, int m0, int n0, int tid) {
    constexpr int RQ = ROWS / 4, CSTEP = NT / RQ;
    const int rq = tid % RQ, col0 = tid / RQ;
    const int m = m0 + 4 * rq;
    if (m >= a.M) return;
    const int ml = m + 3 < a.M ? m + 3 : a.M - 1;
    const int s0 = a.tok_seq[m], t0 = a.tok_t[m];
    const bool run = m + 3 < a.M && a.tok_seq[ml] == s0;
    const bool wide = run && (((t0 | a.Tmax) & 3) == 0);
    int sq[4], tq[4];
    if (!run) {
#pragma unroll
        for (int q = 0; q < 4; ++q) { const int mq = m + q < a.M ? m + q : a.M - 1; sq[q] = a.tok_seq[mq]; tq[q] = a.tok_t[mq]; }
    }
#pragma unroll 4
    for (int i = 0; i < 128 / CSTEP; ++i) {
        const int col = col0 + i * CSTEP;
        const int n = n0 + col;
        if (n >= a.N) break;
        f32x4 v = *(const f32x4*)(ctT + col * (ROWS + 4) + 4 * rq);
        if (a.bias) {
            const float b = a.bias[n];
#pragma unroll
            for (int q = 0; q < 4; ++q) v[q] += b;
        }
        const int c = n - 2 * a.D, hd = c >> 6, d = c & 63;
        if constexpr (F32) {
            if (a.kv_planes) {
                if (run && wide) {
                    pf_store_planes4(a.vcache, a.kv_planes, (((size_t)s0 * a.H + hd) * 64 + d) * a.Tmax + t0, v);
                } else {
#pragma unroll
                    for (int q = 0; q < 4; ++q)
                        if (m + q < a.M) {
                            const size_t o = run ? (((size_t)s0 * a.H + hd) * 64 + d) * a.Tmax + t0 + q : (((size_t)sq[q] * a.H + hd) * 64 + d) * a.Tmax + tq[q];
                            pf_store_planes1(a.vcache, a.kv_planes, o, v[q]);
                        }
                }
                continue;
            }
            if (run) {
                float* vt = (float*)a.vcache + (((size_t)s0 * a.H + hd) * 64 + d) * a.Tmax + t0;
                if (wide) *(f32x4*)vt = v;
                else { vt[0] = v[0]; vt[1] = v[1]; vt[2] = v[2]; vt[3] = v[3]; }
            } else {
#pragma unroll
                for (int q = 0; q < 4; ++q)
                    if (m + q < a.M) ((float*)a.vcache)[(((size_t)sq[q] * a.H + hd) * 64 + d) * a.Tmax + tq[q]] = v[q];
            }
            continue;
        }
        const v2u_t pk = pf_cvt4(v);
        if (run) {
            u16* vt = (u16*)a.vcache + (((size_t)s0 * a.H + hd) * 64 + d) * a.Tmax + t0;
            if (wide) {
                *(v2u_t*)vt = pk;
            } else {
                vt[0] = (u16)(pk.x & 0xffffu); vt[1] = (u16)(pk.x >> 16); vt[2] = (u16)(pk.y & 0xffffu); vt[3] = (u16)(pk.y >> 16);
            }
        } else {
            const u16 e[4] = {(u16)(pk.x & 0xffffu), (u16)(pk.x >> 16), (u16)(pk.y & 0xffffu), (u16)(pk.y >> 16)};
#pragma unroll
            for (int q = 0; q < 4; ++q)
                if (m + q < a.M) ((u16*)a.vcache)[(((size_t)sq[q] * a.H + hd) * 64 + d) * a.Tmax + tq[q]] = e[q];
        }
    }
}

static inline bool pf_vec_ok(const GemmArgs& a) {
    return (a.N % 4 == 0) && (a.ldo % 4 == 0 || (a.epi != EPI_STORE_F32 && a.epi != EPI_RESIDUAL && a.epi != EPI_RESIDUAL_SRC && a.epi != EPI_GELU_ACT)) && (a.D % 4 == 0);
}
static inline bool pf_f32_ok(const GemmArgs& a) {
    return a.K % 32 == 0 && a.lda % 4 == 0 && a.nsplit == 1 && a.epi != EPI_PARTIAL && pf_vec_ok(a) && (((uintptr_t)a.A) & 15) == 0;
}
```

indextts_amd/csrc/gemm_x3.hip:

```cpp
#include "gemm_tile.h"

#define X3_LDS PF_LDS
#define X3_LDS_ONE (96 * 1024)

typedef const __attribute__((address_space(1))) char* pf_gptr_t;
__device__ __forceinline__ pf_gptr_t pf_uni(const char* p) {
    const uint64_t u = (uint64_t)p;
    const uint32_t lo = __builtin_amdgcn_readfirstlane((uint32_t)u), hi = __builtin_amdgcn_readfirstlane((uint32_t)(u >> 32));
    return (pf_gptr_t)(((uint64_t)hi << 32) | lo);
}

__device__ __forceinline__ void x3_split8(const f32x4 p0, const f32x4 p1, v4u& H, v4u& M, v4u& L) {
    const float x[8] = {p0[0], p0[1], p0[2], p0[3], p1[0], p1[1], p1[2], p1[3]};
#pragma unroll
    for (int i = 0; i < 4; ++i) {
        const float a = x[2 * i], b = x[2 * i + 1];
        const uint32_t h = pf_cvt2(a, b);
        const float ra = a - __uint_as_float(h << 16), rb = b - __uint_as_float(h & 0xffff0000u);
        const uint32_t m = pf_cvt2(ra, rb);
        const float sa = ra - __uint_as_float(m << 16), sb = rb - __uint_as_float(m & 0xffff0000u);
        H[i] = h; M[i] = m; L[i] = pf_cvt2(sa, sb);
    }
}

template <int EPI, bool CONV = false, int NPROD = 8, bool SCHED = true, bool APL = false>
__global__ __launch_bounds__(256, 2) void gemm_x3_kernel(GemmArgs a) {
    extern __shared__ __attribute__((aligned(16))) char pf_sm[];
    const int lane = threadIdx.x & 63, w = __builtin_amdgcn_readfirstlane(threadIdx.x >> 6);
    const int wr = w >> 1, wc = w & 1;
    const int n_mt = (a.M + PF_BM - 1) / PF_BM, n_nt = (a.N + PF_BN - 1) / PF_BN;
    const int total = n_mt * n_nt, per = (total + 7) >> 3;
    const int t = (int)(blockIdx.x & 7) * per + (int)(blockIdx.x >> 3);
    if (t >= total) return;
    const int g0 = t / (PF_GM * n_nt), first_m = g0 * PF_GM;
    const int gm = (n_mt - first_m) < PF_GM ? (n_mt - first_m) : PF_GM;
    const int r = t - g0 * PF_GM * n_nt;
    const int bn = r / gm, bm = first_m + (r - bn * gm);
    const int m0 = bm * PF_BM, nt0 = bn * (PF_BN / 16);
    const int nk = a.K >> 5;
    const int ntiles = (a.N + 15) >> 4;

    constexpr int STAGE = APL ? 24576 : 16384;
    const char* asrc[APL ? 6 : 4];
    uint32_t aoff[APL ? 6 : 4];
    const char* abase = (const char*)a.A + (size_t)m0 * a.lda * (APL ? 2 : 4);
    int cv_t[4], cv_T[4];
    const char* cv_base[4];
    const char* cv_zero[4];
    const int cv_kpt = CONV ? a.conv_W / 32 : 1;
    const int cv_left = CONV ? (a.conv_taps - 1) * a.conv_dil - ((a.conv_taps - 1) * a.conv_dil) / 2 : 0;
    if constexpr (APL) {
#pragma unroll
        for (int i = 0; i < 6; ++i) {
            const int pl = i >> 1, c = w + 4 * (i & 1);
            int m = m0 + c * 16 + (lane >> 2);
            m = m < a.M ? m : a.M - 1;
            const int piece = (lane & 3) ^ ((lane >> 4) & 3);
            asrc[i] = (const char*)a.A + ((size_t)pl * a.a_planes + (size_t)m * a.lda) * 2 + piece * 16;
            aoff[i] = (uint32_t)(m - m0) * (uint32_t)a.lda * 2u + piece * 16;
        }
    } else {
#pragma unroll
    for (int i = 0; i < 4; ++i) {
        const int c = w * 4 + i;
        const int row_t = c * 8 + (lane >> 3), row16 = row_t & 15;
        const int piece = (lane & 7) ^ ((row16 >> 1) & 7);
        int m = m0 + row_t;
        m = m < a.M ? m : a.M - 1;
        asrc[i] = (const char*)a.A + (size_t)m * a.lda * 4 + piece * 16;
        aoff[i] = (uint32_t)(m - m0) * (uint32_t)a.lda * 4u + piece * 16;
        if constexpr (CONV) {
            const int sq = a.tok_seq[m];
            cv_t[i] = a.tok_t[m];
            cv_T[i] = a.seq_T[sq];
            cv_base[i] = (const char*)a.A + (size_t)a.seq_start[sq] * a.lda * 4 + piece * 16;
            cv_zero[i] = (const char*)a.zero_row + piece * 16;
        }
    }
    }
    const char* wbase[4];
    const uint32_t lane16 = lane * 16;
#pragma unroll
    for (int nt = 0; nt < 4; ++nt) {
        int ntile = nt0 + wc * 4 + nt;
        ntile = ntile < ntiles ? ntile : ntiles - 1;
        wbase[nt] = (const char*)a.Wp + (size_t)ntile * nk * 3072;
    }
    auto issue_a = [&](int kt, int buf) {
        char* base = pf_sm + buf * STAGE;
        if constexpr (APL) {
#pragma unroll
            for (int i = 0; i < 6; ++i)
                __builtin_amdgcn_global_load_lds((const __attribute__((address_space(1))) void*)(pf_uni(abase + (size_t)(i >> 1) * a.a_planes * 2 + (size_t)kt * 64) + aoff[i]),
                                                 (__attribute__((address_space(3))) void*)(base + (i >> 1) * 8192 + (w + 4 * (i & 1)) * 1024), 16, 0, 0);
            return;
        }
        int tap = 0, rem = kt;
        if constexpr (CONV) { tap = kt / cv_kpt; rem = kt - tap * cv_kpt; }
#pragma unroll
        for (int i = 0; i < 4; ++i) {
            const char* ap = asrc[i] + (size_t)kt * 128;
            if constexpr (CONV) {
                const int maxpad = cv_left;
                const int Tv = cv_T[i] <= maxpad ? maxpad + 1 : cv_T[i];
                int p = cv_t[i] + tap * a.conv_dil - cv_left;
                p = p < 0 ? -p : p;
                p = p >= Tv ? 2 * (Tv - 1) - p : p;
                const bool ok = p >= 0 && p < cv_T[i];
                ap = ok ? cv_base[i] + ((size_t)p * a.lda + (size_t)rem * 32) * 4 : cv_zero[i];
            }
            if constexpr (CONV)
                __builtin_amdgcn_global_load_lds((const __attribute__((address_space(1))) void*)ap,
                                                 (__attribute__((address_space(3))) void*)(base + (w * 4 + i) * 1024), 16, 0, 0);
            else
                __builtin_amdgcn_global_load_lds((const __attribute__((address_space(1))) void*)(pf_uni(abase + (size_t)kt * 128) + aoff[i]),
                                                 (__attribute__((address_space(3))) void*)(base + (w * 4 + i) * 1024), 16, 0, 0);
        }
    };
    auto load_w = [&](int kt, v4u (&bw)[4][3]) {
#pragma unroll
        for (int nt = 0; nt < 4; ++nt)
#pragma unroll
            for (int p = 0; p < 3; ++p) bw[nt][p] = *(const __attribute__((address_space(1))) v4u*)(pf_uni(wbase[nt] + (size_t)kt * 3072) + lane16 + p * 1024);
    };

    f32x4 acc[4][4];
#pragma unroll
    for (int i = 0; i < 4; ++i)
#pragma unroll
        for (int j = 0; j < 4; ++j) acc[i][j] = f32x4{0.f, 0.f, 0.f, 0.f};

    const int row16 = lane & 15, kg = lane >> 4;
    int a_off[2];
#pragma unroll
    for (int s2 = 0; s2 < 2; ++s2) {
        const int pos = (s2 * 4 + kg) ^ ((row16 >> 1) & 7);
        a_off[s2] = (row16 >> 3) * 1024 + ((row16 & 7) * 8 + pos) * 16;
    }
    const int a_wave = wr * 4 * 2048;
    const int a_off_pl = (row16 * 4 + (kg ^ ((row16 >> 2) & 3))) * 16;

    auto ktile = [&](int kt, v4u (&bw)[4][3], v4u (&bn_)[4][3]) {
        asm volatile("s_waitcnt vmcnt(0)" ::: "memory");
        __syncthreads();
        if (kt + 1 < nk) {
            issue_a(kt + 1, (kt + 1) & 1);
            load_w(kt + 1, bn_);
        }
        const char* base = pf_sm + (kt & 1) * STAGE;
        v4u ap[3], an[3];
        if constexpr (APL) {
#pragma unroll
            for (int pl = 0; pl < 3; ++pl) ap[pl] = *(const v4u*)(base + pl * 8192 + wr * 4096 + a_off_pl);
        } else {
            const f32x4 p0 = *(const f32x4*)(base + a_wave + a_off[0]);
            const f32x4 p1 = *(const f32x4*)(base + a_wave + a_off[1]);
            x3_split8(p0, p1, ap[0], ap[1], ap[2]);
        }
#pragma unroll
        for (int mt = 0; mt < 4; ++mt) {
            if (mt < 3) {
                if constexpr (APL) {
#pragma unroll
                    for (int pl = 0; pl < 3; ++pl) an[pl] = *(const v4u*)(base + pl * 8192 + wr * 4096 + (mt + 1) * 1024 + a_off_pl);
                } else {
                const f32x4 p0 = *(const f32x4*)(base + a_wave + (mt + 1) * 2048 + a_off[0]);
                const f32x4 p1 = *(const f32x4*)(base + a_wave + (mt + 1) * 2048 + a_off[1]);
                x3_split8(p0, p1, an[0], an[1], an[2]);
                }
            }
            constexpr int PA[8] = {2, 1, 2, 0, 1, 1, 0, 0};
            constexpr int PB[8] = {1, 2, 0, 2, 1, 0, 1, 0};
#pragma unroll
            for (int q = 8 - NPROD; q < 8; ++q)
#pragma unroll
                for (int nt = 0; nt < 4; ++nt)
                    acc[mt][nt] = __builtin_amdgcn_mfma_f32_16x16x32_bf16(__builtin_bit_cast(bf16x8_t, ap[PA[q]]),
                                                                          __builtin_bit_cast(bf16x8_t, bw[nt][PB[q]]), acc[mt][nt], 0, 0, 0);
            if (APL && mt < 3) {
                __builtin_amdgcn_sched_group_barrier(0x100, 3, 0);
                __builtin_amdgcn_sched_group_barrier(0x008, 4 * NPROD, 0);
            }
            if (!APL && SCHED && mt < 3) {
                __builtin_amdgcn_sched_group_barrier(0x100, 2, 0);
#pragma unroll
                for (int i = 0; i < 2 * NPROD; ++i) {
                    __builtin_amdgcn_sched_group_barrier(0x008, 2, 0);
                    __builtin_amdgcn_sched_group_barrier(0x002, 3, 0);
                }
            }
            if (mt < 3) { ap[0] = an[0]; ap[1] = an[1]; ap[2] = an[2]; }
        }
    };
    v4u bw0[4][3], bw1[4][3];
    issue_a(0, 0);
    load_w(0, bw0);
    for (int kt = 0; kt < nk; kt += 2) {
        ktile(kt, bw0, bw1);
        if (kt + 1 < nk) ktile(kt + 1, bw1, bw0);
    }
    __syncthreads();
    float* ct = (float*)pf_sm;
    const int g = lane >> 4, c16 = lane & 15;
    if (EPI == EPI_QKV_ROPE && a.D % 128 == 0 && nt0 * 16 >= 2 * a.D) {
#pragma unroll
        for (int mt = 0; mt < 4; ++mt)
#pragma unroll
            for (int nt = 0; nt < 4; ++nt) *(f32x4*)(ct + (wc * 64 + nt * 16 + c16) * 132 + wr * 64 + mt * 16 + g * 4) = acc[mt][nt];
        __syncthreads();
        pf_store_vt<128, 256, true>(a, ct, m0, nt0 * 16, threadIdx.x);
        return;
    }
#pragma unroll
    for (int mt = 0; mt < 4; ++mt)
#pragma unroll
        for (int nt = 0; nt < 4; ++nt)
#pragma unroll
            for (int rr = 0; rr < 4; ++rr)
                ct[(wr * 64 + mt * 16 + g * 4 + rr) * 128 + ((wc * 64 + nt * 16 + c16) ^ (g << 4))] = acc[mt][nt][rr];
    int* meta = (int*)(pf_sm + 65536);
    pf_stage_meta<EPI, 128>(a, meta, m0, threadIdx.x);
    __syncthreads();
    pf_store_tile<EPI, 128, 256, true>(a, ct, meta, m0, nt0 * 16, threadIdx.x);
}


#define X3W8_STAGE (16384 + 24576)
#define X3W8_LDS (2 * X3W8_STAGE)
template <int EPI, bool CONV = false>
__global__ __launch_bounds__(512, 2) void gemm_x3w8_kernel(GemmArgs a) {
    extern __shared__ __attribute__((aligned(16))) char pf_sm[];
    constexpr int NPROD = 6;
    const int lane = threadIdx.x & 63, w = __builtin_amdgcn_readfirstlane(threadIdx.x >> 6);
    const int wr = w >> 1, wc = w & 1;
    const int n_mt = (a.M + PF_BM - 1) / PF_BM, n_nt = (a.N + PF_BN - 1) / PF_BN;
    const int total = n_mt * n_nt, per = (total + 7) >> 3;
    const int t = (int)(blockIdx.x & 7) * per + (int)(blockIdx.x >> 3);
    if (t >= total) return;
    const int g0 = t / (PF_GM * n_nt), first_m = g0 * PF_GM;
    const int gm = (n_mt - first_m) < PF_GM ? (n_mt - first_m) : PF_GM;
    const int r = t - g0 * PF_GM * n_nt;
    const int bn = r / gm, bm = first_m + (r - bn * gm);
    const int m0 = bm * PF_BM, nt0 = bn * (PF_BN / 16);
    const int nk = a.K >> 5;
    const int ntiles = (a.N + 15) >> 4;

    const char* asrc[2];
    uint32_t aoff[2];
    const char* abase = (const char*)a.A + (size_t)m0 * a.lda * 4;
    int cv_t[2], cv_T[2];
    const char* cv_base[2];
    const char* cv_zero[2];
    const int cv_kpt = CONV ? a.conv_W / 32 : 1;
    const int cv_left = CONV ? (a.conv_taps - 1) * a.conv_dil - ((a.conv_taps - 1) * a.conv_dil) / 2 : 0;
#pragma unroll
    for (int i = 0; i < 2; ++i) {
        const int c = w * 2 + i;
        const int row_t = c * 8 + (lane >> 3), row16 = row_t & 15;
        const int piece = (lane & 7) ^ ((row16 >> 1) & 7);
        int m = m0 + row_t;
        m = m < a.M ? m : a.M - 1;
        asrc[i] = (const char*)a.A + (size_t)m * a.lda * 4 + piece * 16;
        aoff[i] = (uint32_t)(m - m0) * (uint32_t)a.lda * 4u + piece * 16;
        if constexpr (CONV) {
            const int sq = a.tok_seq[m];
            cv_t[i] = a.tok_t[m];
            cv_T[i] = a.seq_T[sq];
            cv_base[i] = (const char*)a.A + (size_t)a.seq_start[sq] * a.lda * 4 + piece * 16;
            cv_zero[i] = (const char*)a.zero_row + piece * 16;
        }
    }
    const char* wdma[3];
    const uint32_t lane16 = lane * 16;
#pragma unroll
    for (int i = 0; i < 3; ++i) {
        const int q = w + 8 * i;
        int ntile = nt0 + q / 3;
        ntile = ntile < ntiles ? ntile : ntiles - 1;
        wdma[i] = (const char*)a.Wp + (size_t)ntile * nk * 3072 + (q % 3) * 1024;
    }
    auto issue = [&](int kt, int buf) {
        char* base = pf_sm + buf * X3W8_STAGE;
        int tap = 0, rem = kt;
        if constexpr (CONV) { tap = kt / cv_kpt; rem = kt - tap * cv_kpt; }
#pragma unroll
        for (int i = 0; i < 2; ++i) {
            if constexpr (CONV) {
                const int maxpad = cv_left;
                const int Tv = cv_T[i] <= maxpad ? maxpad + 1 : cv_T[i];
                int p = cv_t[i] + tap * a.conv_dil - cv_left;
                p = p < 0 ? -p : p;
                p = p >= Tv ? 2 * (Tv - 1) - p : p;
                const bool ok = p >= 0 && p < cv_T[i];
                const char* ap = ok ? cv_base[i] + ((size_t)p * a.lda + (size_t)rem * 32) * 4 : cv_zero[i];
                __builtin_amdgcn_global_load_lds((const __attribute__((address_space(1))) void*)ap,
                                                 (__attribute__((address_space(3))) void*)(base + (w * 2 + i) * 1024), 16, 0, 0);
            } else {
                (void)asrc;
                __builtin_amdgcn_global_load_lds((const __attribute__((address_space(1))) void*)(pf_uni(abase + (size_t)kt * 128) + aoff[i]),
                                                 (__attribute__((address_space(3))) void*)(base + (w * 2 + i) * 1024), 16, 0, 0);
            }
        }
#pragma unroll
        for (int i = 0; i < 3; ++i)
            __builtin_amdgcn_global_load_lds((const __attribute__((address_space(1))) void*)(pf_uni(wdma[i] + (size_t)kt * 3072) + lane16),
                                             (__attribute__((address_space(3))) void*)(base + 16384 + (w + 8 * i) * 1024), 16, 0, 0);
    };

    f32x4 acc[2][4];
#pragma unroll
    for (int i = 0; i < 2; ++i)
#pragma unroll
        for (int j = 0; j < 4; ++j) acc[i][j] = f32x4{0.f, 0.f, 0.f, 0.f};

    const int row16 = lane & 15, kg = lane >> 4;
    int a_off[2];
#pragma unroll
    for (int s2 = 0; s2 < 2; ++s2) {
        const int pos = (s2 * 4 + kg) ^ ((row16 >> 1) & 7);
        a_off[s2] = (row16 >> 3) * 1024 + ((row16 & 7) * 8 + pos) * 16;
    }
    const int a_wave = wr * 2 * 2048;

    issue(0, 0);
    for (int kt = 0; kt < nk; ++kt) {
        asm volatile("s_waitcnt vmcnt(0)" ::: "memory");
        __syncthreads();
        if (kt + 1 < nk) issue(kt + 1, (kt + 1) & 1);
        const char* base = pf_sm + (kt & 1) * X3W8_STAGE;
        v4u bw[4][3];
#pragma unroll
        for (int nt = 0; nt < 4; ++nt)
#pragma unroll
            for (int p = 0; p < 3; ++p) bw[nt][p] = *(const v4u*)(base + 16384 + ((wc * 4 + nt) * 3 + p) * 1024 + lane16);
        v4u ap[3], an[3];
        {
            const f32x4 p0 = *(const f32x4*)(base + a_wave + a_off[0]);
            const f32x4 p1 = *(const f32x4*)(base + a_wave + a_off[1]);
            x3_split8(p0, p1, ap[0], ap[1], ap[2]);
        }
#pragma unroll
        for (int mt = 0; mt < 2; ++mt) {
            if (mt < 1) {
                const f32x4 p0 = *(const f32x4*)(base + a_wave + (mt + 1) * 2048 + a_off[0]);
                const f32x4 p1 = *(const f32x4*)(base + a_wave + (mt + 1) * 2048 + a_off[1]);
                x3_split8(p0, p1, an[0], an[1], an[2]);
            }
            constexpr int PA[8] = {2, 1, 2, 0, 1, 1, 0, 0};
            constexpr int PB[8] = {1, 2, 0, 2, 1, 0, 1, 0};
#pragma unroll
            for (int q = 8 - NPROD; q < 8; ++q)
#pragma unroll
                for (int nt = 0; nt < 4; ++nt)
                    acc[mt][nt] = __builtin_amdgcn_mfma_f32_16x16x32_bf16(__builtin_bit_cast(bf16x8_t, ap[PA[q]]),
                                                                          __builtin_bit_cast(bf16x8_t, bw[nt][PB[q]]), acc[mt][nt], 0, 0, 0);
            if (mt < 1) {
                __builtin_amdgcn_sched_group_barrier(0x100, 2, 0);
#pragma unroll
                for (int i = 0; i < 2 * NPROD; ++i) {
                    __builtin_amdgcn_sched_group_barrier(0x008, 2, 0);
                    __builtin_amdgcn_sched_group_barrier(0x002, 3, 0);
                }
                ap[0] = an[0]; ap[1] = an[1]; ap[2] = an[2];
            }
        }
    }
    __syncthreads();
    float* ct = (float*)pf_sm;
    const int g = lane >> 4, c16 = lane & 15;
    if (EPI == EPI_QKV_ROPE && a.D % 128 == 0 && nt0 * 16 >= 2 * a.D) {
#pragma unroll
        for (int mt = 0; mt < 2; ++mt)
#pragma unroll
            for (int nt = 0; nt < 4; ++nt) *(f32x4*)(ct + (wc * 64 + nt * 16 + c16) * 132 + wr * 32 + mt * 16 + g * 4) = acc[mt][nt];
        __syncthreads();
        pf_store_vt<128, 512, true>(a, ct, m0, nt0 * 16, threadIdx.x);
        return;
    }
#pragma unroll
    for (int mt = 0; mt < 2; ++mt)
#pragma unroll
        for (int nt = 0; nt < 4; ++nt)
#pragma unroll
            for (int rr = 0; rr < 4; ++rr)
                ct[(wr * 32 + mt * 16 + g * 4 + rr) * 128 + ((wc * 64 + nt * 16 + c16) ^ (g << 4))] = acc[mt][nt][rr];
    int* meta = (int*)(pf_sm + 65536);
    pf_stage_meta<EPI, 128>(a, meta, m0, threadIdx.x);
    __syncthreads();
    pf_store_tile<EPI, 128, 512, true>(a, ct, meta, m0, nt0 * 16, threadIdx.x);
}

template <int EPI, bool CONV = false>
static int launch_gemm_x3_e(const GemmArgs& a, hipStream_t st) {
    const int n_mt = ceil_div(a.M, PF_BM), n_nt = ceil_div(a.N, PF_BN);
    const int per = ceil_div(n_mt * n_nt, 8);
    const int nprod = itts_opt(OPT_X3_PRODUCTS) == 6 ? 6 : 8;
    const bool sched = itts_opt(OPT_X3_SCHED) != 0;
    static ItPerDevice<bool> attr_set_pd;
    bool& attr_set = attr_set_pd.cur();
    if (!attr_set) {
        HIP_TRY(hipFuncSetAttribute((const void*)gemm_x3_kernel<EPI, CONV, 8, true>, hipFuncAttributeMaxDynamicSharedMemorySize, X3_LDS_ONE));
        HIP_TRY(hipFuncSetAttribute((const void*)gemm_x3_kernel<EPI, CONV, 6, true>, hipFuncAttributeMaxDynamicSharedMemorySize, X3_LDS_ONE));
        HIP_TRY(hipFuncSetAttribute((const void*)gemm_x3_kernel<EPI, CONV, 8, false>, hipFuncAttributeMaxDynamicSharedMemorySize, X3_LDS_ONE));
        HIP_TRY(hipFuncSetAttribute((const void*)gemm_x3_kernel<EPI, CONV, 6, false>, hipFuncAttributeMaxDynamicSharedMemorySize, X3_LDS_ONE));
        attr_set = true;
    }
    const dim3 grid(per * 8), blk(256);
    const size_t lds = ((nprod == 6 && sched) || itts_opt(OPT_X3_PIN) == 0) ? X3_LDS : X3_LDS_ONE;
    if constexpr (!CONV && (EPI == EPI_QKV_ROPE || EPI == EPI_SWIGLU)) {
        if (a.a_planes) {
            if (nprod != 6 || !sched) { itts_set_error("gemm (f32x3): the plane-operand form exists for the shipped variant only (6 products, interleaved)"); return ITTS_ERR_ARG; }
            static ItPerDevice<bool> apl_set_pd;
            bool& apl_set = apl_set_pd.cur();
            if (!apl_set) {
                HIP_TRY(hipFuncSetAttribute((const void*)gemm_x3_kernel<EPI, CONV, 6, true, true>, hipFuncAttributeMaxDynamicSharedMemorySize, X3_LDS_ONE));
                apl_set = true;
            }
            gemm_note_path(GP_X3_4W_APLANES);
            hipLaunchKernelGGL((gemm_x3_kernel<EPI, CONV, 6, true, true>), grid, blk, lds, st, a);
            HIP_TRY(hipGetLastError());
            return ITTS_OK;
        }
    } else if (a.a_planes) { itts_set_error("gemm (f32x3): plane operands are supported for the wqkv / SwiGLU GEMMs only"); return ITTS_ERR_ARG; }
    if (nprod == 6 && sched && itts_opt(OPT_X3_WAVES) == 8 && itts_opt(OPT_X3_PIN) == 0) {
        static ItPerDevice<bool> w8_set_pd;
        bool& w8_set = w8_set_pd.cur();
        if (!w8_set) {
            HIP_TRY(hipFuncSetAttribute((const void*)gemm_x3w8_kernel<EPI, CONV>, hipFuncAttributeMaxDynamicSharedMemorySize, X3W8_LDS));
            w8_set = true;
        }
        gemm_note_path(GP_X3_8W);
        hipLaunchKernelGGL((gemm_x3w8_kernel<EPI, CONV>), grid, dim3(512), X3W8_LDS, st, a);
        HIP_TRY(hipGetLastError());
        return ITTS_OK;
    }
    gemm_note_path(nprod == 6 ? GP_X3_4W_P6 : GP_X3_4W_P8);
    if (nprod == 6 && sched) hipLaunchKernelGGL((gemm_x3_kernel<EPI, CONV, 6, true>), grid, blk, lds, st, a);
    else if (nprod == 6) hipLaunchKernelGGL((gemm_x3_kernel<EPI, CONV, 6, false>), grid, blk, lds, st, a);
    else if (sched) hipLaunchKernelGGL((gemm_x3_kernel<EPI, CONV, 8, true>), grid, blk, lds, st, a);
    else hipLaunchKernelGGL((gemm_x3_kernel<EPI, CONV, 8, false>), grid, blk, lds, st, a);
    HIP_TRY(hipGetLastError());
    return ITTS_OK;
}

int launch_gemm_x3(const GemmArgs& a, hipStream_t st) {
    if (!pf_f32_ok(a)) {
        itts_set_error("gemm (f32x3): needs K %% 32 == 0, lda %% 4 == 0, N / ldo / D %% 4 == 0, 16-byte aligned rows, no split-K (M=%d N=%d K=%d lda=%d epi=%d)",
                       a.M, a.N, a.K, a.lda, a.epi);
        return ITTS_ERR_ARG;
    }
    if (a.epi == EPI_GATE && a.conv_taps > 0 &&
        (a.conv_W % 32 || a.K != a.conv_taps * a.conv_W || a.lda != a.conv_W || !a.tok_seq || !a.tok_t || !a.seq_start || !a.seq_T || !a.zero_row)) {
        itts_set_error("gemm tap mode (f32x3): need conv_W %% 32 == 0, K == taps * conv_W, lda == conv_W and the sequence tables");
        return ITTS_ERR_ARG;
    }
    switch (a.epi) {
        case EPI_STORE_F32: return launch_gemm_x3_e<EPI_STORE_F32>(a, st);
        case EPI_RESIDUAL: return launch_gemm_x3_e<EPI_RESIDUAL>(a, st);
        case EPI_RESIDUAL_SRC:
            if (!a.res_src || a.res_src == a.out_f32) { itts_set_error("gemm (f32x3): EPI_RESIDUAL_SRC needs a residual source other than the output"); return ITTS_ERR_ARG; }
            return launch_gemm_x3_e<EPI_RESIDUAL_SRC>(a, st);
        case EPI_SWIGLU: return launch_gemm_x3_e<EPI_SWIGLU>(a, st);
        case EPI_GATE: return a.conv_taps > 0 ? launch_gemm_x3_e<EPI_GATE, true>(a, st) : launch_gemm_x3_e<EPI_GATE>(a, st);
        case EPI_QKV_ROPE: return launch_gemm_x3_e<EPI_QKV_ROPE>(a, st);
        case EPI_WN_RS: return launch_gemm_x3_e<EPI_WN_RS>(a, st);
        default: itts_set_error("gemm (f32x3): unsupported epilogue %d", a.epi); return ITTS_ERR_ARG;
    }
}


int gemm_x3_occupancy(int* blocks) {
    int n = 0;
    (void)hipFuncSetAttribute((const void*)gemm_x3_kernel<EPI_RESIDUAL, false, 6, true>, hipFuncAttributeMaxDynamicSharedMemorySize, X3_LDS);
    const hipError_t e = hipOccupancyMaxActiveBlocksPerMultiprocessor(&n, (const void*)gemm_x3_kernel<EPI_RESIDUAL, false, 6, true>, 256, X3_LDS);
    if (e != hipSuccess) { itts_set_error("occupancy query: %s", hipGetErrorString(e)); return ITTS_ERR_HIP; }
    *blocks = n;
    return ITTS_OK;
}
```

indextts_amd/csrc/gpt_kernels.h:

```cpp
#pragma once
#include "common.h"

enum { PREC_F32 = 0, PREC_BF16 = 1,
       PREC_F32X3 = 2 };

struct LnArgs {
    float* x;
    const float* partial;
    int nsplit;
    const float* bias_prev;
    const float* g1; const float* b1;
    const float* g2; const float* b2;
    void* out;
    int out_f32;
    int rows, D;
    int in_row_mul, in_row_add;
    float eps;
};
int launch_ln(const LnArgs& a, int prec, hipStream_t st);

enum { EPI_STORE_F32 = 0, EPI_GELU_ACT = 1, EPI_PARTIAL = 2, EPI_RESIDUAL = 3, EPI_QKV = 4,
       EPI_SWIGLU = 5,
       EPI_GATE = 6,
       EPI_QKV_ROPE = 7,
       EPI_WN_RS = 8,
       EPI_RESIDUAL_SRC = 9 };
struct GemmArgs {
    const void* A; int lda;
    const void* Wp;
    const float* bias;
    int M, N, K;
    int nsplit;
    int epi;
    float* out_f32; int ldo;
    void* out_act;
    float* partial;
    float* qbuf; void* kcache; void* vcache;
    const int* pos_ptr; int S, H, Tmax, D;
    const int* pos_shift;
    size_t a_planes;
    int kb_slice;
    int dma_rot;
    const float* ln_x; float* ln_x_out; const float* ln_partial; const float* ln_bias_prev; const float* ln_g; const float* ln_b; float ln_eps;
    const int* tok_seq; const int* tok_t; const int* seq_len; const float* rope; const float* gvec;
    float* out2; int wn_first, wn_last;
    int conv_taps, conv_dil, conv_W;
    const int* seq_start; const int* seq_T; const void* zero_row;
    void* out_act2;
    int seq_mul;
    const int* seq_map;
    size_t kv_planes;
    const float* res_src;
    const int* res_map;
};
int launch_gemm(const GemmArgs& a, int prec, bool prefill, hipStream_t st);
int launch_gemm_x3(const GemmArgs& a, hipStream_t st);
int gemm_x3_occupancy(int* blocks);
bool gemm_decode_ln_ok(int M, int K, int epi);
int launch_gemm_decode_ln(const GemmArgs& a, hipStream_t st);
int gemm_tile_occupancy(int prec, int* blocks);

enum GemmPath {
    GP_NONE = -1,
    GP_BF16_TILE128, GP_BF16_TILE128_NOVEC, GP_BF16_TILE256, GP_BF16_TILE256X128, GP_BF16_REG_PREFILL,
    GP_BF16_SLAB_MT1, GP_BF16_SLAB_MT2, GP_BF16_SLAB_MT4_NT1, GP_BF16_SLAB_MT4_NT2, GP_BF16_SLAB_MT4_NT4,
    GP_BF16_REG_DECODE_MT1, GP_BF16_REG_DECODE_MT2, GP_BF16_REG_DECODE_MT4,
    GP_F32_TILE, GP_F32_REG_PREFILL, GP_F32_REG_DECODE_MT1, GP_F32_REG_DECODE_MT2, GP_F32_REG_DECODE_MT4,
    GP_X3_4W_P6, GP_X3_4W_P8, GP_X3_4W_APLANES, GP_X3_8W,
    GP_BF16_LN_DECODE_4W, GP_BF16_LN_DECODE_WIDE_NT2, GP_BF16_LN_DECODE_WIDE_NT4,
    GP_COUNT
};
void gemm_note_path(int path);
int gemm_last_path();
const char* gemm_path_name(int path);

struct AttnArgs {
    const float* qbuf;
    const void* kcache; const void* vcache;
    const int* pad;
    const int* row_map;
    const int* row_map_alt;
    const int* step_ptr;
    const int* pos_ptr;
    const int* pos_shift;
    void* out;
    int nseq, H, nq, Tmax, D;
    int seq_mul;
    const int* seq_map;
};
int launch_attention(const AttnArgs& a, int prec, hipStream_t st);

enum AttnPath {
    AP_NONE = -1,
    AP_STREAMS_F32_W4, AP_STREAMS_F32_W4_RMAP, AP_STREAMS_F32_W8, AP_STREAMS_F32_W8_RMAP, AP_STREAMS_F32_W16, AP_STREAMS_F32_W16_RMAP,
    AP_STREAMS_BF16_W4, AP_STREAMS_BF16_W4_RMAP, AP_STREAMS_BF16_W8, AP_STREAMS_BF16_W8_RMAP, AP_STREAMS_BF16_W16, AP_STREAMS_BF16_W16_RMAP,
    AP_PREFILL_MFMA_F32, AP_PREFILL_MFMA_BF16,
    AP_COUNT
};
int attention_last_path();
const char* attention_path_name(int path);

struct RowSampling {
    int do_sample, top_k, min_keep;
    float top_p, temperature, rep_penalty, typical_mass;
    int stream;
    unsigned long long seed;
};
struct LogitsFilters {
    int min_new_tokens, min_length;
    int ngram;
    int decay_start;
    int n_decay;
    int has_mask;
    int prompt_len;
    int start_mel;
    float min_p;
    float epsilon, eta;
    const unsigned char* mask;
    const float* decay;
};
struct SampleArgs {
    const float* logits;
    unsigned char* seen;
    unsigned char* finished;
    long long* tokens;
    const int* step_ptr;
    const double* uniforms;
    unsigned long long seed;
    int B, V, max_new;
    int do_sample, top_k, min_keep;
    float top_p, temperature, rep_penalty;
    float typical_mass;
    int stop_token;
    const float* mel_emb; const float* mel_pos; float* x_next; int D; int pos_offset; int n_mel_pos;
    int* adv_state;
    const unsigned long long* seed_ptr;
// ... 56 lines not shown
```

indextts_amd/csrc/gpt_kernels.hip:

```cpp
#include "gemm_tile.h"


enum { LN_PARTIAL = 1, LN_BIAS = 2, LN_SECOND = 4 };

template <int NV, int FLAGS>
__device__ __forceinline__ void ln_row(const float* __restrict__ xr, float* __restrict__ xw, const float* __restrict__ pp, size_t ps,
                                       const float* __restrict__ bias_prev, const float* __restrict__ ga1, const float* __restrict__ be1,
                                       const float* __restrict__ ga2, const float* __restrict__ be2, int D, float eps, int lane, f32x4 (&v)[NV]) {
#pragma clang fp contract(off)
    f32x4 p0[NV], p1[NV], p2[NV], p3[NV], bp[NV], g1[NV], b1[NV], g2[NV], b2[NV];
#pragma unroll
    for (int i = 0; i < NV; ++i) {
        const int e = 4 * lane + 256 * i;
        v[i] = *(const f32x4*)(xr + e);
        if constexpr (FLAGS & LN_PARTIAL) {
            p0[i] = *(const f32x4*)(pp + e); p1[i] = *(const f32x4*)(pp + ps + e);
            p2[i] = *(const f32x4*)(pp + 2 * ps + e); p3[i] = *(const f32x4*)(pp + 3 * ps + e);
        }
        if constexpr (FLAGS & LN_BIAS) bp[i] = *(const f32x4*)(bias_prev + e);
        g1[i] = *(const f32x4*)(ga1 + e);
        b1[i] = *(const f32x4*)(be1 + e);
        if constexpr (FLAGS & LN_SECOND) { g2[i] = *(const f32x4*)(ga2 + e); b2[i] = *(const f32x4*)(be2 + e); }
    }
    __builtin_amdgcn_sched_barrier(0);
// ... 1535 lines not shown

bool gemm_decode_ln_ok(int M, int K, int epi) {
    return M >= 1 && M <= 16 && (K == 256 || K == 512 || K == 1280) && (epi == EPI_QKV || epi == EPI_GELU_ACT || epi == EPI_STORE_F32);
}

int launch_gemm_decode_ln(const GemmArgs& a, hipStream_t st) {
    if (!gemm_decode_ln_ok(a.M, a.K, a.epi) || a.nsplit != 1 || !a.ln_x || !a.ln_g || !a.ln_b) {
        itts_set_error("gemm_decode_ln: unsupported call (M=%d K=%d epi=%d nsplit=%d)", a.M, a.K, a.epi, a.nsplit);
        return ITTS_ERR_ARG;
    }
#define LN_GEMM_CASE(NV_)                                                                                        \
    case NV_: return a.epi == EPI_QKV ? launch_gemm_decode_ln_e<NV_, EPI_QKV>(a, st) : a.epi == EPI_GELU_ACT ? launch_gemm_decode_ln_e<NV_, EPI_GELU_ACT>(a, st) \
                                                                                                               : launch_gemm_decode_ln_e<NV_, EPI_STORE_F32>(a, st);
    switch (a.K / 256) { LN_GEMM_CASE(1) LN_GEMM_CASE(2) LN_GEMM_CASE(5) default: break; }
#undef LN_GEMM_CASE
    return ITTS_ERR_ARG;
}

template <bool BF16, int MT, int NT, bool KSPLIT>
static int launch_gemm_cfg(const GemmArgs& a, hipStream_t st) {
    const int ntiles = (a.N + 15) / 16;
    const int per_block = KSPLIT ? NT : 4 * NT;
    dim3 grid(ceil_div(ntiles, per_block), ceil_div(a.M, MT * 16), a.nsplit);
    const size_t lds = KSPLIT ? (size_t)4 * MT * NT * 64 * 16 + (MT >= 4 ? (size_t)MT * 16 * (20 * 64 + 16) : 0) : 0;
    static_assert(!KSPLIT || MT == 1 || MT == 2 || MT == 4, "register-path decode geometries: 16 / 32 / 64 rows per block");
    gemm_note_path(!KSPLIT ? (BF16 ? GP_BF16_REG_PREFILL : GP_F32_REG_PREFILL)
                           : BF16 ? (MT == 1 ? GP_BF16_REG_DECODE_MT1 : MT == 2 ? GP_BF16_REG_DECODE_MT2 : GP_BF16_REG_DECODE_MT4)
                                  : (MT == 1 ? GP_F32_REG_DECODE_MT1 : MT == 2 ? GP_F32_REG_DECODE_MT2 : GP_F32_REG_DECODE_MT4));
    hipLaunchKernelGGL((gemm_kernel<BF16, MT, NT, KSPLIT>), grid, dim3(256), lds, st, a);
    HIP_TRY(hipGetLastError());
    return ITTS_OK;
}

template <bool BF16>
static int launch_gemm_t(const GemmArgs& a, bool prefill, hipStream_t st) {
    if (prefill) {
        const bool old_path = itts_opt(OPT_PREFILL_GEMM) == 0;
        if (BF16 && !old_path && a.K % PF_BK == 0 && a.lda % 8 == 0 && a.nsplit == 1 && a.epi != EPI_PARTIAL) return launch_gemm_prefill(a, st);
        if constexpr (!BF16) {
            const bool f32_reg = itts_opt(OPT_F32_TILE) == 0;
            const bool fused = a.epi > EPI_QKV || a.out_act2 != nullptr;
            if (pf_f32_ok(a) && (fused || !f32_reg)) return launch_gemm_prefill_f32(a, st);
        }
        if (a.epi > EPI_QKV || a.out_act2) { itts_set_error("gemm: epilogue %d / shadow output needs a tile kernel (bf16: K %% 64 == 0, lda %% 8 == 0; f32: K %% 32 == 0, lda %% 4 == 0, N / ldo / D %% 4 == 0)", a.epi); return ITTS_ERR_ARG; }
        return launch_gemm_cfg<BF16, 8, 2, false>(a, st);
    }
    if constexpr (BF16) {
        const bool old_path = itts_opt(OPT_DECODE_GEMM) == 0;
        if (!old_path && ceil_div(a.K / 32, a.nsplit) <= 40 && a.lda % 8 == 0 && (a.K / 32) % (2 * a.nsplit) == 0) {
            const int rc = launch_gemm_decode64(a, st);
            if (rc >= 0) return rc;
        }
    }
    if (a.M <= 16) return launch_gemm_cfg<BF16, 1, 1, true>(a, st);
    if (a.M <= 32) return launch_gemm_cfg<BF16, 2, 1, true>(a, st);
    return launch_gemm_cfg<BF16, 4, 1, true>(a, st);
}

int gemm_tile_occupancy(int prec, int* blocks) {
    int n = 0;
    hipError_t e;
    if (prec == PREC_F32) {
        (void)hipFuncSetAttribute((const void*)gemm_prefill_kernel<EPI_RESIDUAL, false, true, true>, hipFuncAttributeMaxDynamicSharedMemorySize, PF_LDS);
        e = hipOccupancyMaxActiveBlocksPerMultiprocessor(&n, (const void*)gemm_prefill_kernel<EPI_RESIDUAL, false, true, true>, 256, PF_LDS);
    } else if (prec == PREC_F32X3) {
        return gemm_x3_occupancy(blocks);
    } else {
        (void)hipFuncSetAttribute((const void*)gemm_prefill_kernel<EPI_RESIDUAL, false, true, false>, hipFuncAttributeMaxDynamicSharedMemorySize, PF_LDS);
        e = hipOccupancyMaxActiveBlocksPerMultiprocessor(&n, (const void*)gemm_prefill_kernel<EPI_RESIDUAL, false, true, false>, 256, PF_LDS);
    }
    if (e != hipSuccess) { itts_set_error("occupancy query: %s", hipGetErrorString(e)); return ITTS_ERR_HIP; }
    *blocks = n;
    return ITTS_OK;
}

int launch_gemm(const GemmArgs& a, int prec, bool prefill, hipStream_t st) {
    if (a.M <= 0 || a.N <= 0) return ITTS_OK;
    const int KB = prec == PREC_F32 ? 16 : 32;
    if (a.K % KB || a.nsplit < 1 || (a.K / KB) < a.nsplit) {
        itts_set_error("gemm: K=%d must be a multiple of %d and >= nsplit=%d blocks", a.K, KB, a.nsplit);
        return ITTS_ERR_ARG;
    }
    if (a.nsplit > 1 && a.epi != EPI_PARTIAL) { itts_set_error("gemm: split-K needs EPI_PARTIAL"); return ITTS_ERR_ARG; }
    if (prec == PREC_F32X3) return launch_gemm_x3(a, st);
    return prec == PREC_BF16 ? launch_gemm_t<true>(a, prefill, st) : launch_gemm_t<false>(a, prefill, st);
}

template <bool BF16>
__device__ __forceinline__ float exp_sel(float x) { return BF16 ? __expf(x) : expf(x); }

#define ATTN_STREAMS 16
template <bool BF16, int NW, bool RMAP>
__global__ __launch_bounds__(NW * 64) void attn_kernel(AttnArgs a) {
    constexpr int LPK = BF16 ? 8 : 16;
    constexpr int DPL = 64 / LPK;
    constexpr int KPW = 64 / LPK;
    constexpr int CH = 64;
    constexpr int LPC = CH / KPW;
    constexpr int UB = 8;
    __shared__ float sm_m[ATTN_STREAMS], sm_l[ATTN_STREAMS], sm_acc[ATTN_STREAMS][64];
    const int lane = threadIdx.x & 63, w = threadIdx.x >> 6;
    const int b = blockIdx.x / a.H, h = blockIdx.x - b * a.H;
    const int qi = blockIdx.y;
    const int sm = a.seq_mul > 1 ? a.seq_mul : 1;
    const int pb = a.seq_map ? a.seq_map[b] : b * sm;
    int last = *a.pos_ptr + qi - (a.pos_shift ? a.pos_shift[pb] : 0);
    last = last < a.Tmax ? last : a.Tmax - 1;
    const int first = a.pad ? a.pad[pb] : 0;
    const int sub = lane % LPK, grp = lane / LPK;
    const size_t qrow = (size_t)b * a.nq + qi;
    const int* rmap = a.row_map;
    if constexpr (RMAP) {
        if (a.row_map_alt && a.step_ptr && (*a.step_ptr & 1)) rmap = a.row_map_alt;
    }

    float q[DPL];
#pragma unroll
    for (int d = 0; d < DPL; ++d) q[d] = a.qbuf[qrow * a.D + h * 64 + sub * DPL + d];

    for (int r = w; r < ATTN_STREAMS; r += NW) {
        float m_run = -INFINITY, l_run = 0.f, acc[DPL];
#pragma unroll
        for (int d = 0; d < DPL; ++d) acc[d] = 0.f;
        for (int c = r; first + c * CH <= last; c += ATTN_STREAMS) {
            const int tb = first + c * CH;
#pragma unroll
            for (int h0 = 0; h0 < LPC; h0 += UB) {
                if (tb + h0 * KPW > last) break;
                bool okv[UB];
                int tcv[UB], prowv[UB];
                v4u kraw[UB], vraw[UB];
#pragma unroll
                for (int u = 0; u < UB; ++u) {
                    const int t = tb + (h0 + u) * KPW + grp;
                    okv[u] = t <= last;
                    tcv[u] = okv[u] ? t : last;
                    if constexpr (RMAP) prowv[u] = rmap[(size_t)b * a.Tmax + tcv[u]];
                    else prowv[u] = pb;
                }
#pragma unroll
                for (int u = 0; u < UB; ++u) {
                    const size_t off = (((size_t)prowv[u] * a.H + h) * a.Tmax + tcv[u]) * 64 + sub * DPL;
                    if constexpr (BF16) {
                        kraw[u] = *(const v4u*)((const u16*)a.kcache + off);
                        vraw[u] = *(const v4u*)((const u16*)a.vcache + off);
                    } else {
                        kraw[u] = *(const v4u*)((const float*)a.kcache + off);
                        vraw[u] = *(const v4u*)((const float*)a.vcache + off);
                    }
                }
                __builtin_amdgcn_sched_barrier(0);
#pragma unroll
                for (int u = 0; u < UB; ++u) {
                    float kf[DPL], vf[DPL];
                    if constexpr (BF16) {
#pragma unroll
                        for (int i = 0; i < 4; ++i) {
                            kf[2 * i] = __uint_as_float(kraw[u][i] << 16);
                            kf[2 * i + 1] = __uint_as_float(kraw[u][i] & 0xffff0000u);
                            vf[2 * i] = __uint_as_float(vraw[u][i] << 16);
                            vf[2 * i + 1] = __uint_as_float(vraw[u][i] & 0xffff0000u);
                        }
                    } else {
#pragma unroll
                        for (int i = 0; i < 4; ++i) { kf[i] = __uint_as_float(kraw[u][i]); vf[i] = __uint_as_float(vraw[u][i]); }
                    }
// ... 1160 lines not shown
```

indextts_amd/csrc/options.hip:

```cpp
#include <atomic>
#include <stdlib.h>
#include <string.h>

#include "../../include/indextts_hip.h"
#include "common.h"

namespace {
struct OptDef {
    const char* name;
    int def, lo, hi;
    const char* doc;
    const char* allowed = nullptr;
};
const OptDef kDefs[OPT_COUNT] = {
    {"decode_fuse_ln", 1, 0, 2, "GPT decode: LayerNorm (+ split-K reduce, bias, residual) inside the consuming GEMM -- 1: steps of 1-8 rows (measured faster), 2: up to 16 rows (measured slower above 8, kept for the A/B record), 0: separate ln_kernel launches; bitwise equal"},
    {"decode_gemm", 1, 0, 1, "bf16 decode GEMMs on the LDS-DMA slab kernel (0: register-path gemm_kernel; bitwise equal)"},
    {"decode_rot", 1, 0, 1, "per-block rotation of the slab DMA issue order in the decode GEMM (same bytes, same LDS image)"},
    {"decode_wnt", 0, 0, 1, "non-temporal policy on the decode GEMM's weight stream"},
    {"decode_nt", 0, 0, 4, "force the n-tiles per block of the 64-row decode GEMM (0: smallest that fits one round of blocks)", "0,1,2,4"},
    {"prefill_gemm", 1, 0, 1, "bf16 prefill GEMMs on the LDS-DMA tile kernels (0: register-path gemm_kernel; bitwise equal)"},
    {"tile256", -1, -1, 2, "bf16 tile GEMM: -1 pick by shape, 0 always 128x128, 1 always 256x256, 2 always 256x128 (bitwise equal)"},
    {"f32_tile", 1, 0, 1, "f32 GEMMs with plain epilogues on the f32-MFMA tile kernel (0: register-path kernel; bitwise equal)"},
    {"x3_products", 6, 6, 8, "plane products per f32 product of the fp32x3 GEMMs and attention: 6 (hh, hm, mh, hl, lh, mm; drops m*l and l*m, 2^-24 |ab| each: measured error vs f64 <= the native f32-MFMA kernels' on every benchmarked shape) or 8 (every term down to 2^-24 |ab|; two blocks per CU like the default since the packed-RoPE fix -- option x3_pin = 1 restores round 4's one-block pin as a diagnostic)", "6,8"},
    {"x3_sched", 1, 0, 1, "fp32x3 GEMM: interleave the operand split with the MFMAs (0: split as a burst; bitwise equal)"},
    {"x3_attn", 1, 0, 1, "fp32x3 s2mel: attention products on bf16 planes too (K / V^T written as three planes by the wqkv epilogue, flash_attn_x3_kernel); 0: the f32-MFMA flash kernel"},
    {"sample_radix", -1, -1, 1, "top-k threshold: -1 per-kernel default (radix select in sample_kernel, ballot bisection in the beam kernels), 0 bisection, 1 radix select (identical ids)"},
    {"gpt_compact", 1, 0, 1, "row compaction of ragged decode batches (0 disables it for every handle; identical ids)"},
    {"attn_waves", 0, 0, 16, "waves per block of the KV-cache attention kernel: 0 pick by shape, else 4 / 8 / 16 (the 16 canonical key streams are mapped onto them; bitwise equal)", "0,4,8,16"},
    {"s2mel_fused", 1, 0, 2, "s2mel: fused GEMM epilogues, sampled when a handle is created -- 1: fused, 0: separate element-wise kernels (2: round 4's spelling of 'the bf16 wqkv epilogue fused too'; the same as 1 since the RoPE fix of round 5)"},
    {"fa_qs", 0, 0, 4, "bf16 flash attention: query sub-tiles per wave (0: pick by shape)", "0,1,2,4"},
    {"f32_attn_scalar", 0, 0, 1, "f32 s2mel attention on the one-wave-per-query reference kernel (the A/B path of the f32 flash kernel)"},
    {"fa32_qs", 2, 1, 2, "f32 flash attention: query sub-tiles per wave"},
    {"aa_act", 2, 0, 2, "anti-aliased activation kernel variant (2: swizzled LDS tiles)"},
    {"conv_bm", 0, 0, 128, "force the co-tile height of conv_mfma_kernel (0: pick by channel count)", "0,32,64,96,128"},
    {"h3_kernel", 1, 0, 1, "f16x3 vocoder conv: 1 window kernel, 0 two-stage kernel"},
    {"decode_ln_nt", 2, 2, 4, "LayerNorm-fused decode GEMM at 5-16 rows (weights on waves 0-3, LayerNorm on waves 4-7): n-tiles per block, 2 or 4 (bitwise equal)", "2,4"},
    {"x3_aplanes", 0, 0, 1, "fp32x3 s2mel: the adaptive-RMSNorm outputs as three bf16 planes in fragment order, wqkv / w1|w3 GEMMs without an operand split (bitwise equal)"},
    {"x3_pin", 0, 0, 1, "fp32x3 GEMM: 1 pins the variants that are not the default one (8 products, burst split) to one block per CU -- round 4's workaround for their run-to-run differences, kept as a diagnostic; not needed since the RoPE fix of round 5 (DESIGN.md section 9)"},
    {"prefill_attn", -1, -1, 1, "attention of S > 1 passes (prefill, latent pass): -1 causal MFMA kernel in the bf16 mode, canonical-stream kernel in the f32 parity mode; 0 canonical-stream kernel (one block per query) always; 1 MFMA kernel in both precisions"},
    {"voc_act_planes", 1, 0, 1, "vocoder, bf16x3 conv mode: the anti-aliased activation in front of an x3 conv writes the conv's three operand planes itself (aa_act_planes_kernel); 0: f32 activation + split pass (bit-identical planes)"},
    {"x3_waves", 8, 4, 8, "fp32x3 GEMM: waves per 128 x 128 block -- 8 (4 x 2, wave tile 32 x 64, weights through LDS: four waves per SIMD at two blocks per CU; 64-utterance solve 314.7 vs 323.0 ms per Euler step, profiles/r06k) or 4 (2 x 2, wave tile 64 x 64, weights in registers: round 5's kernel); bitwise equal", "4,8"},
    {"s2mel_prune_last", 1, 0, 1, "fp32x3 s2mel solve with a tail layout: the LAST DiT layer's attention runs the queries of the tail rows only (keys / values: every frame) and writes the tail layout, its wo / FFN norm / w1|w3 / w2 stages run on the tail rows (residual gathered by a row map in the wo epilogue); the x_in GEMM reads its residual from const_in instead of a copy of it; 0: every row, copy first (bitwise equal)"},
    {"x3_attn_skip", 1, 0, 1, "fp32x3 flash attention: a last key tile with <= 32 valid keys skips the MFMAs of its fully masked half, and a wave whose 32 queries are all out of range only stages its share of K / V^T (0: full tiles, every wave computes; bitwise equal)"},
};
std::atomic<int> g_val[OPT_COUNT];
std::atomic<unsigned> g_epoch{1};
std::atomic<bool> g_init{false};

void ensure_init() {
    if (g_init.load(std::memory_order_acquire)) return;
    static std::atomic_flag once = ATOMIC_FLAG_INIT;
    if (!once.test_and_set()) {
        for (int i = 0; i < OPT_COUNT; ++i) g_val[i].store(kDefs[i].def, std::memory_order_relaxed);
        g_init.store(true, std::memory_order_release);
    } else {
        while (!g_init.load(std::memory_order_acquire)) {}
    }
}
int find(const char* name) {
    if (!name) return -1;
    for (int i = 0; i < OPT_COUNT; ++i)
        if (strcmp(kDefs[i].name, name) == 0) return i;
    return -1;
}
}

int itts_opt(int id) {
    ensure_init();
    return g_val[id].load(std::memory_order_relaxed);
}
unsigned itts_opt_epoch() { return g_epoch.load(std::memory_order_relaxed); }

extern "C" int itts_set_option(const char* name, int value) {
    ensure_init();
    const int i = find(name);
    if (i < 0) { itts_set_error("set_option: unknown option '%s'", name ? name : "(null)"); return ITTS_ERR_ARG; }
    if (value < kDefs[i].lo || value > kDefs[i].hi) {
        itts_set_error("set_option: %s = %d outside [%d, %d]", name, value, kDefs[i].lo, kDefs[i].hi);
        return ITTS_ERR_ARG;
    }
    if (kDefs[i].allowed) {
        bool ok = false;
        for (const char* p = kDefs[i].allowed; *p;) {
            char* end;
            const long v = strtol(p, &end, 10);
            ok |= v == value;
            p = *end == ',' ? end + 1 : end;
        }
        if (!ok) { itts_set_error("set_option: %s = %d is not one of {%s}", name, value, kDefs[i].allowed); return ITTS_ERR_ARG; }
    }
    if (g_val[i].exchange(value) != value) g_epoch.fetch_add(1);
    return ITTS_OK;
}
extern "C" int itts_get_option(const char* name, int* value) {
    ensure_init();
    const int i = find(name);
    if (i < 0 || !value) { itts_set_error("get_option: unknown option '%s'", name ? name : "(null)"); return ITTS_ERR_ARG; }
    *value = g_val[i].load();
    return ITTS_OK;
}
extern "C" int itts_reset_options(void) {
    ensure_init();
    bool changed = false;
    for (int i = 0; i < OPT_COUNT; ++i) changed |= g_val[i].exchange(kDefs[i].def) != kDefs[i].def;
    if (changed) g_epoch.fetch_add(1);
    return ITTS_OK;
}
extern "C" int itts_option_count(void) { return OPT_COUNT; }
extern "C" const char* itts_option_name(int index) { return (index >= 0 && index < OPT_COUNT) ? kDefs[index].name : nullptr; }
extern "C" const char* itts_option_doc(int index) { return (index >= 0 && index < OPT_COUNT) ? kDefs[index].doc : nullptr; }
extern "C" int itts_option_default(int index) { return (index >= 0 && index < OPT_COUNT) ? kDefs[index].def : 0; }
```

indextts_amd/gpt.py:

```python
import ctypes as C
from typing import List, Dict, Optional, Sequence

import torch
import torch.nn.functional as F

from . import _lib


_UNSUPPORTED_GENERATE_KWARGS = frozenset((
    "encoder_no_repeat_ngram_size", "num_beam_groups",
    "diversity_penalty", "penalty_alpha", "early_stopping", "stopping_criteria", "prefix_allowed_tokens_fn", "constraints",
    "force_words_ids", "forced_bos_token_id", "forced_eos_token_id",
    "encoder_repetition_penalty", "renormalize_logits",
    "guidance_scale", "sequence_bias", "typical_p", "assistant_model", "negative_prompt_ids"))

_LOGITS_FILTER_KWARGS = ("no_repeat_ngram_size", "bad_words_ids", "min_length", "min_new_tokens", "suppress_tokens", "begin_suppress_tokens",
                         "epsilon_cutoff", "eta_cutoff", "exponential_decay_length_penalty", "min_p")
_SUPPORTED_GENERATE_KWARGS = ("do_sample, num_beams, top_p, top_k, temperature, repetition_penalty, length_penalty, typical sampling, "
                              + ", ".join(_LOGITS_FILTER_KWARGS))


def logits_filters(kwargs: dict, vocab: int, stop_token: int, max_new_tokens: int, num_beams: int = 1, who: str = "generate",
                   prompt_len: Optional[int] = None):
    g = lambda k: kwargs.get(k)
# ... 1318 lines not shown
        except Exception:
            pass


class UnifiedVoiceV1(UnifiedVoice):
    _ALLOW_ENCODER_CONDITIONING = True
    _HOST_TENSORS = ("mel_embedding.weight", "mel_pos_embedding.emb.weight", "text_embedding.weight",
                     "text_pos_embedding.emb.weight")
    _OPTIONAL_HOST_TENSORS = ()

    def __init__(self, *args, condition_type="conformer_perceiver", conditioning_fn=None, **kw):
        kw.setdefault("spk_cond_mode", "encoder")
        super().__init__(*args, condition_type=condition_type, **kw)
        self.condition_type = condition_type
        self.conditioning_fn = conditioning_fn

    def get_conditioning(self, speech_conditioning_input, cond_mel_lengths=None):
        if self.conditioning_fn is None:
            raise NotImplementedError("v1 conditioning encoder (Conformer + Perceiver) is outside the engine: set "
                                      "UnifiedVoiceV1.conditioning_fn or pass conds_latent=")
        return self.conditioning_fn(speech_conditioning_input, cond_mel_lengths)

    def prepare_gpt_inputs(self, conditional_latents, text_inputs):
        return super().prepare_gpt_inputs(conditional_latents, text_inputs, None)

    def inference_speech(self, speech_conditioning_mel, text_inputs, cond_mel_lengths=None, input_tokens=None,
                         num_return_sequences=1, max_generate_length=None, typical_sampling=False, typical_mass=.9,
                         conds_latent=None, uniforms=None, **hf_generate_kwargs):
        if input_tokens is not None or num_return_sequences != 1:
            raise NotImplementedError("input_tokens / num_return_sequences > 1 are not used by the v1 pipeline")
        if typical_sampling and not (typical_mass > 0.0 and typical_mass < 1.0):
            raise ValueError(f"`typical_mass` has to be a float > 0 and < 1, but is {typical_mass}")
        if conds_latent is None:
            if speech_conditioning_mel.ndim == 2:
                speech_conditioning_mel = speech_conditioning_mel.unsqueeze(0)
            if cond_mel_lengths is None:
                cond_mel_lengths = torch.tensor([speech_conditioning_mel.shape[-1]], device=speech_conditioning_mel.device)
            conds_latent = self.get_conditioning(speech_conditioning_mel, cond_mel_lengths)
        input_ids, inputs_embeds, attention_mask = self.prepare_gpt_inputs(conds_latent, text_inputs)
        max_new = (self.max_mel_tokens - 1) if max_generate_length is None else int(max_generate_length)
        hf = dict(hf_generate_kwargs)
        _reject_logits_processor(hf)
        return self.generate(inputs_embeds, attention_mask, max_new, uniforms=uniforms,
                             typical_mass=float(typical_mass) if typical_sampling else 0.0, **hf)

    def forward(self, speech_conditioning_latent, text_inputs, text_lengths, mel_codes, wav_lengths, cond_mel_lengths=None,
                types=None, text_first=True, raw_mels=None, return_attentions=False, return_latent=False,
                clip_inputs=False, conds_latent=None):
        if not return_latent or not text_first or raw_mels is not None or return_attentions or clip_inputs:
            raise NotImplementedError("only the return_latent=True, text_first inference form is on the engine path")
        if conds_latent is None:
            conds_latent = self.get_conditioning(speech_conditioning_latent, cond_mel_lengths)
        if types is not None:
            text_inputs = text_inputs * (1 + types).unsqueeze(-1)
        wl = torch.as_tensor(wav_lengths)
        mel_codes_lengths = torch.ceil(wl / self.mel_length_compression).long() + 1
        b = text_inputs.shape[0]
        conds = conds_latent.expand(b, -1, -1) if conds_latent.shape[0] == 1 and b > 1 else conds_latent
        return self.forward_latent(conds, text_inputs, torch.as_tensor(text_lengths), mel_codes, mel_codes_lengths)

    __call__ = forward


def pack_gemm_weight(w_kn: torch.Tensor, precision: int, transposed: bool = False) -> torch.Tensor:
    w = w_kn.detach().to("cpu", torch.float32).contiguous()
    K, N = (w.shape[1], w.shape[0]) if transposed else (w.shape[0], w.shape[1])
    L = _lib.lib()
    out = torch.empty(L.itts_packed_gemm_bytes(K, N, precision), dtype=torch.uint8)
    _lib.check(L.itts_pack_gemm_weight(_lib.ptr(w), K, N, int(transposed), precision, _lib.ptr(out)), "itts_pack_gemm_weight")
    return out


def gemm(a: torch.Tensor, w_packed: torch.Tensor, bias: Optional[torch.Tensor], N: int, precision: int,
         prefill_tiles: bool = False) -> torch.Tensor:
    M, K = a.shape
    out = torch.empty(M, N, dtype=torch.float32, device=a.device)
    with _lib.on_device(a.device):
        _lib.check(_lib.lib().itts_gemm_forward(_lib.ptr(a.contiguous()), _lib.ptr(w_packed), _lib.ptr(bias), _lib.ptr(out),
                                                M, N, K, precision, int(prefill_tiles), 0, _lib.stream_ptr(a.device)),
                   "itts_gemm_forward")
        return out


def linear_f32(x: torch.Tensor, weight: torch.Tensor, bias: Optional[torch.Tensor], cache: Optional[dict] = None, key=None) -> torch.Tensor:
    N, K = weight.shape
    if K % 16:
        return F.linear(x, weight.to(x.device), None if bias is None else bias.to(x.device))
    packed = cache.get(key) if cache is not None and key is not None else None
    if packed is None or packed.device != x.device:
        packed = pack_gemm_weight(weight, 0, transposed=True).to(x.device)
        if cache is not None and key is not None:
            cache[key] = packed
    lead = x.shape[:-1]
    a = x.reshape(-1, K).to(torch.float32).contiguous()
    out = gemm(a, packed, None if bias is None else bias.to(x.device, torch.float32).contiguous(), N, 0)
    return out.reshape(*lead, N)


def _spk_proj(x: torch.Tensor, w64: torch.Tensor, b64: torch.Tensor) -> torch.Tensor:
    y = x.detach().to("cpu", torch.float64) @ w64.t() + b64
    return y.to(torch.float32).to(x.device)


def gemm_ln(x, g, b, w_packed, bias, N: int, partial=None, bias_prev=None, eps=1e-5):
    M, K = x.shape
    out = torch.empty(M, N, dtype=torch.float32, device=x.device)
    x_out = torch.empty_like(x) if partial is not None else None
    with _lib.on_device(x.device):
        _lib.check(_lib.lib().itts_gemm_ln_forward(_lib.ptr(x.contiguous()), _lib.ptr(partial), _lib.ptr(bias_prev), _lib.ptr(g), _lib.ptr(b),
                                                   float(eps), _lib.ptr(w_packed), _lib.ptr(bias), _lib.ptr(out), _lib.ptr(x_out), M, N, K,
                                                   _lib.stream_ptr(x.device)), "itts_gemm_ln_forward")
    return out, x_out


def layernorm(x, g, b, g2=None, b2=None, eps=1e-5):
    rows, D = x.shape
    out = torch.empty_like(x)
    with _lib.on_device(x.device):
        _lib.check(_lib.lib().itts_layernorm_forward(_lib.ptr(x.contiguous()), _lib.ptr(g), _lib.ptr(b), _lib.ptr(g2),
                                                     _lib.ptr(b2), _lib.ptr(out), rows, D, float(eps), _lib.stream_ptr(x.device)),
                   "itts_layernorm_forward")
        return out
```

Before: 142.1.

## Drop redundant f32 shadow copies and fuse skip GEMM pairs in fp32x3 s2mel

Adds two default-on options for the fp32x3 s2mel path. The first stops writing f32 shadow copies that duplicate the epilogue output: the saved U-ViT skip becomes the stream buffer itself through out-of-place w2/wo GEMMs, and downstream GEMMs read the f32 outputs directly, so the workspace no longer needs WXA. The second merges each skip_in and skip_linear pair (a store GEMM followed by a read-add-store GEMM) into a single two-source GEMM that accumulates over the K tiles of both operands. This cuts memory traffic and kernel launches per DiT step, at the cost of more complex buffer rotation and slightly different low bits in the fused accumulation.

```diff
diff --git a/include/indextts_hip.h b/include/indextts_hip.h
--- a/include/indextts_hip.h
+++ b/include/indextts_hip.h
@@ -214,6 +214,8 @@
 const char* itts_gemm_path_name(int index);
 int itts_gemm_forward(const void* A, const void* Wp, const float* bias, float* out, int M, int N, int K, int precision,
                       int prefill_tiles, int gelu, void* stream);
+int itts_gemm_cat_forward(const void* A, int lda, const void* Wp, const void* A2, int lda2, const void* Wp2, const float* bias, float* out,
+                          int M, int N, int K1, int K2, int precision, void* stream);
 int itts_layernorm_forward(const float* x, const float* gamma, const float* beta, const float* gamma2,
                            const float* beta2, float* out, int rows, int D, float eps, void* stream);
 const char* itts_attention_last_path(void);
diff --git a/indextts_amd/_lib.py b/indextts_amd/_lib.py
--- a/indextts_amd/_lib.py
+++ b/indextts_amd/_lib.py
@@ -198,6 +198,7 @@
     "itts_gemm_path_count": (C.c_int, []),
     "itts_gemm_path_name": (C.c_char_p, [C.c_int]),
     "itts_gemm_forward": (C.c_int, [vp, vp, vp, vp, C.c_int, C.c_int, C.c_int, C.c_int, C.c_int, C.c_int, vp]),
+    "itts_gemm_cat_forward": (C.c_int, [vp, C.c_int, vp, vp, C.c_int, vp, vp, vp, C.c_int, C.c_int, C.c_int, C.c_int, C.c_int, vp]),
     "itts_attention_last_path": (C.c_char_p, []),
     "itts_attention_path_count": (C.c_int, []),
     "itts_attention_path_name": (C.c_char_p, [C.c_int]),
diff --git a/indextts_amd/csrc/capi_gpt.hip b/indextts_amd/csrc/capi_gpt.hip
--- a/indextts_amd/csrc/capi_gpt.hip
+++ b/indextts_amd/csrc/capi_gpt.hip
@@ -1714,6 +1714,18 @@
     return launch_gemm(g, precision, prefill_tiles != 0, (hipStream_t)stream);
 }
 
+extern "C" int itts_gemm_cat_forward(const void* A, int lda, const void* Wp, const void* A2, int lda2, const void* Wp2, const float* bias, float* out,
+                                     int M, int N, int K1, int K2, int precision, void* stream) {
+    if (!A || !Wp || !A2 || !Wp2 || !out) { itts_set_error("gemm_cat_forward: null pointer"); return ITTS_ERR_ARG; }
+    if (precision != PREC_F32X3) { itts_set_error("gemm_cat_forward: precision %d (the two-source GEMM exists in the fp32x3 mode only)", precision); return ITTS_ERR_ARG; }
+    if (K1 <= 0 || K2 <= 0 || K1 % 32 || K2 % 32) { itts_set_error("gemm_cat_forward: K1=%d, K2=%d must be positive multiples of 32", K1, K2); return ITTS_ERR_ARG; }
+    GemmArgs g{};
+    g.A = A; g.lda = lda; g.Wp = Wp; g.A2 = A2; g.lda2 = lda2; g.Wp2 = Wp2; g.k_split = K1;
+    g.bias = bias; g.M = M; g.N = N; g.K = K1 + K2; g.nsplit = 1; g.D = N;
+    g.epi = EPI_STORE_F32; g.out_f32 = out; g.ldo = N;
+    return launch_gemm(g, precision, true, (hipStream_t)stream);
+}
+
 extern "C" const char* itts_attention_last_path(void) {
     const char* n = attention_path_name(attention_last_path());
     return n ? n : "none";
diff --git a/indextts_amd/csrc/capi_s2mel.hip b/indextts_amd/csrc/capi_s2mel.hip
--- a/indextts_amd/csrc/capi_s2mel.hip
+++ b/indextts_amd/csrc/capi_s2mel.hip
@@ -14,6 +14,8 @@
     if (precision == PREC_F32X3) return true;
     return (precision == PREC_BF16 || precision == PREC_F32) && opt_fused;
 }
+
+static bool s2_dedup(int precision, bool opt_fused) { return precision == PREC_F32X3 && s2_fused(precision, opt_fused) && itts_opt(OPT_S2MEL_DEDUP) != 0; }
 
 struct S2Layer {
     void *w_qkv = 0, *w_o = 0, *w_13 = 0, *w_2 = 0, *w_skip_a = 0, *w_skip_b = 0;
@@ -390,7 +392,7 @@
     w.XA = take(N * Kx * esz);
     w.sk_stride = s_a256(N * H * esz);
     w.SK = take(w.sk_stride * (size_t)(c.depth / 2));
-    w.WXA = take(N * W * esz);
+    w.WXA = s2_dedup(c.precision, h->opt_fused) ? nullptr : take(N * W * esz);
     w.hbp_stride = (N * H + 127) / 128 * 128;
     w.HBP = take(c.precision == PREC_F32X3 ? w.hbp_stride * 6 : 0);
     const size_t kv = (size_t)n_seq * c.num_heads * t_pad * 64 * (c.precision == PREC_F32X3 ? 6 : esz);
@@ -432,8 +434,11 @@
     const bool a_planes = prec == PREC_F32X3 && fused && itts_opt(OPT_X3_APLANES) != 0 && itts_opt(OPT_X3_PRODUCTS) == 6 && itts_opt(OPT_X3_SCHED) != 0 && H % 32 == 0;
     const bool prune_opt = prec == PREC_F32X3 && fused && itts_opt(OPT_S2MEL_PRUNE_LAST) != 0;
     const bool prune_last = prune_opt && x3_attn && tail != nullptr && c.depth > 0;
+    const bool dedup = s2_dedup(prec, h->opt_fused);
+    const bool skip_fuse = prec == PREC_F32X3 && fused && itts_opt(OPT_S2MEL_SKIP_FUSE) != 0;
     int rc;
     float *X = w.X, *X2 = w.X2;
+    float* spare = nullptr;
     const size_t esz = prec == PREC_BF16 ? 2 : 4;
     const size_t kvb = kv_plane * (prec == PREC_F32X3 ? (x3_attn ? 6 : 4) : esz);
 #define S2_TRACE(label, ptr, bytes) do { if (h->trace && (rc = s2_trace(h, st, label, ptr, bytes))) return rc; } while (0)
@@ -453,8 +458,16 @@
         if (i > c.depth / 2) {
             if (!fused && (rc = launch_cast_pad(X, w.HB, N, N, H, H, prec, st))) return rc;
             --n_skip;
-            if ((rc = s2_gemm(h, w.HB, H, L.w_skip_a, L.b_skip, X2, H, N, H, H, EPI_STORE_F32, st))) return rc;
-            if ((rc = s2_gemm(h, w.SK + w.sk_stride * n_skip, H, L.w_skip_b, nullptr, X2, H, N, H, H, EPI_RESIDUAL, st))) return rc;
+            const void* xa = dedup ? (const void*)X : (const void*)w.HB;
+            if (skip_fuse) {
+                GemmArgs g{};
+                g.A = xa; g.lda = H; g.Wp = L.w_skip_a; g.A2 = w.SK + w.sk_stride * n_skip; g.lda2 = H; g.Wp2 = L.w_skip_b; g.k_split = H;
+                g.bias = L.b_skip; g.M = N; g.N = H; g.K = 2 * H; g.nsplit = 1; g.epi = EPI_STORE_F32; g.out_f32 = X2; g.ldo = H; g.D = H;
+                if ((rc = s2_launch_gemm(h, g, st))) return rc;
+            } else {
+                if ((rc = s2_gemm(h, xa, H, L.w_skip_a, L.b_skip, X2, H, N, H, H, EPI_STORE_F32, st))) return rc;
+                if ((rc = s2_gemm(h, w.SK + w.sk_stride * n_skip, H, L.w_skip_b, nullptr, X2, H, N, H, H, EPI_RESIDUAL, st))) return rc;
+            }
             S2_TRACE("skip_in GEMMs -> X", X2, (size_t)N * H * 4);
             float* tmp = X; X = X2; X2 = tmp;
         }
@@ -492,7 +505,14 @@
             g.A = w.AO; g.lda = H; g.Wp = L.w_o; g.M = NL; g.N = H; g.K = H; g.nsplit = 1; g.epi = EPI_RESIDUAL_SRC; g.out_f32 = X2; g.ldo = H; g.D = H;
             g.res_src = X; g.res_map = tail_src;
             if ((rc = s2_launch_gemm(h, g, st))) return rc;
-            float* tmp = X; X = X2; X2 = tmp;
+            if (spare) { X = X2; X2 = spare; spare = nullptr; }
+            else { float* tmp = X; X = X2; X2 = tmp; }
+        } else if (spare) {
+            GemmArgs g{};
+            g.A = w.AO; g.lda = H; g.Wp = L.w_o; g.M = N; g.N = H; g.K = H; g.nsplit = 1; g.epi = EPI_RESIDUAL_SRC; g.out_f32 = spare; g.ldo = H; g.D = H;
+            g.res_src = X;
+            if ((rc = s2_launch_gemm(h, g, st))) return rc;
+            X = spare; spare = nullptr;
         } else if ((rc = s2_gemm(h, w.AO, H, L.w_o, nullptr, X, H, N, H, H, EPI_RESIDUAL, st))) return rc;
         S2_TRACE("wo GEMM -> X", X, (size_t)NL * H * 4);
         if (a_planes) {
@@ -512,10 +532,16 @@
             if ((rc = launch_swiglu(w.BIG, w.FC, NL, I, prec, st))) return rc;
         }
         void* shadow = nullptr;
-        if (fused && i < c.depth / 2) shadow = w.SK + w.sk_stride * n_skip;
-        else if (fused && i + 1 < c.depth && i + 1 > c.depth / 2) shadow = w.HB;
+        if (fused && !dedup && i < c.depth / 2) shadow = w.SK + w.sk_stride * n_skip;
+        else if (fused && !dedup && i + 1 < c.depth && i + 1 > c.depth / 2) shadow = w.HB;
         S2_TRACE("w13 + SwiGLU -> FC", w.FC, (size_t)NL * I * esz);
-        if ((rc = s2_gemm(h, w.FC, I, L.w_2, nullptr, X, H, NL, H, I, EPI_RESIDUAL, st, shadow))) return rc;
+        if (dedup && i < c.depth / 2 && !pruned) {
+            GemmArgs g{};
+            g.A = w.FC; g.lda = I; g.Wp = L.w_2; g.M = NL; g.N = H; g.K = I; g.nsplit = 1; g.epi = EPI_RESIDUAL_SRC; g.ldo = H; g.D = H;
+            g.out_f32 = (float*)(w.SK + w.sk_stride * n_skip); g.res_src = X;
+            if ((rc = s2_launch_gemm(h, g, st))) return rc;
+            spare = X; X = g.out_f32;
+        } else if ((rc = s2_gemm(h, w.FC, I, L.w_2, nullptr, X, H, NL, H, I, EPI_RESIDUAL, st, shadow))) return rc;
         S2_TRACE("w2 GEMM -> X", X, (size_t)NL * H * 4);
         if (i < c.depth / 2) {
             if (!fused && (rc = launch_cast_pad(X, w.SK + w.sk_stride * n_skip, N, N, H, H, prec, st))) return rc;
@@ -534,13 +560,22 @@
     const int NT = tt.n_tok;
     if ((rc = launch_ada_rmsnorm(X, h->g_norm, m_norm, w.HB, NT, H, c.norm_eps, prec, st, tail && !prune_last ? tail_src : nullptr))) return rc;
     S2_TRACE("final ada_rmsnorm -> HB", w.HB, (size_t)NT * H * esz);
-    if ((rc = s2_gemm(h, w.HB, H, h->w_sl_a, h->b_sl, X2, H, NT, H, H, EPI_STORE_F32, st))) return rc;
-    if ((rc = s2_gemm(h, XAt, Kx, h->w_sl_b, nullptr, X2, H, NT, H, Kx, EPI_RESIDUAL, st, fused ? w.HB : nullptr))) return rc;
+    const bool sl_direct = dedup || skip_fuse;
+    if (skip_fuse) {
+        GemmArgs g{};
+        g.A = w.HB; g.lda = H; g.Wp = h->w_sl_a; g.A2 = XAt; g.lda2 = Kx; g.Wp2 = h->w_sl_b; g.k_split = H;
+        g.bias = h->b_sl; g.M = NT; g.N = H; g.K = H + Kx; g.nsplit = 1; g.epi = EPI_STORE_F32; g.out_f32 = X2; g.ldo = H; g.D = H;
+        if ((rc = s2_launch_gemm(h, g, st))) return rc;
+    } else {
+        if ((rc = s2_gemm(h, w.HB, H, h->w_sl_a, h->b_sl, X2, H, NT, H, H, EPI_STORE_F32, st))) return rc;
+        if ((rc = s2_gemm(h, XAt, Kx, h->w_sl_b, nullptr, X2, H, NT, H, Kx, EPI_RESIDUAL, st, fused && !sl_direct ? w.HB : nullptr))) return rc;
+    }
     if (!fused && (rc = launch_cast_pad(X2, w.HB, NT, NT, H, H, prec, st))) return rc;
     S2_TRACE("skip_linear -> X2", X2, (size_t)NT * H * 4);
-    if ((rc = s2_gemm(h, w.HB, H, h->w_c1, h->b_c1, w.WX, W, NT, W, H, EPI_STORE_F32, st, fused ? w.WXA : nullptr))) return rc;
+    const void* x_res = sl_direct ? (const void*)X2 : (const void*)w.HB;
+    if ((rc = s2_gemm(h, x_res, H, h->w_c1, h->b_c1, w.WX, W, NT, W, H, EPI_STORE_F32, st, fused && !dedup ? w.WXA : nullptr))) return rc;
     S2_TRACE("conv1 -> WX", w.WX, (size_t)NT * W * 4);
-    if ((rc = s2_gemm(h, w.HB, H, h->w_rp, h->b_rp, w.RP, W, NT, W, H, EPI_STORE_F32, st))) return rc;
+    if ((rc = s2_gemm(h, x_res, H, h->w_rp, h->b_rp, w.RP, W, NT, W, H, EPI_STORE_F32, st))) return rc;
     int dil = 1;
     for (int i = 0; i < c.wavenet_layers; ++i) {
         const S2Wn& Wn = h->wn[i];
@@ -549,14 +584,14 @@
         const int ro = last ? W : 2 * W;
         if (fused) {
             GemmArgs g{};
-            g.A = w.WXA; g.lda = W; g.Wp = Wn.w_in; g.bias = Wn.b_in; g.M = NT; g.N = 2 * W; g.K = c.wavenet_kernel * W;
+            g.A = dedup ? (const void*)w.WX : (const void*)w.WXA; g.lda = W; g.Wp = Wn.w_in; g.bias = Wn.b_in; g.M = NT; g.N = 2 * W; g.K = c.wavenet_kernel * W;
             g.nsplit = 1; g.epi = EPI_GATE; g.out_act = w.FC; g.gvec = m_gc + (size_t)i * 2 * W; g.D = W;
             g.conv_taps = c.wavenet_kernel; g.conv_dil = dil; g.conv_W = W; g.tok_seq = tt.tok_seq; g.tok_t = tt.tok_t;
             g.seq_start = tt.seq_start; g.seq_T = tt.seq_T; g.zero_row = w.ZR;
             if ((rc = s2_launch_gemm(h, g, st))) return rc;
             GemmArgs r{};
             r.A = w.FC; r.lda = W; r.Wp = Wn.w_rs; r.bias = Wn.b_rs; r.M = NT; r.N = ro; r.K = W; r.nsplit = 1; r.epi = EPI_WN_RS;
-            r.out_f32 = w.WX; r.out2 = w.OUT; r.D = W; r.wn_first = i == 0; r.wn_last = last; r.out_act2 = last ? nullptr : w.WXA;
+            r.out_f32 = w.WX; r.out2 = w.OUT; r.D = W; r.wn_first = i == 0; r.wn_last = last; r.out_act2 = (last || dedup) ? nullptr : w.WXA;
             r.tok_seq = tt.tok_seq; r.tok_t = tt.tok_t; r.seq_len = tt.seq_len;
             S2_TRACE("wavenet in_layer + gate -> FC", w.FC, (size_t)NT * W * esz);
             if ((rc = s2_launch_gemm(h, r, st))) return rc;
@@ -571,10 +606,11 @@
         dil *= c.wavenet_dilation_rate;
     }
     if ((rc = launch_final_ln_mod(w.OUT, w.RP, m_fl, w.HB, tt, W, prec, st))) return rc;
-    if ((rc = s2_gemm(h, w.HB, W, h->w_fl, h->b_fl, w.BIG, W, NT, W, W, EPI_STORE_F32, st, fused ? w.FC : nullptr))) return rc;
+    if ((rc = s2_gemm(h, w.HB, W, h->w_fl, h->b_fl, w.BIG, W, NT, W, W, EPI_STORE_F32, st, fused && !dedup ? w.FC : nullptr))) return rc;
     if (!fused && (rc = launch_cast_pad(w.BIG, w.FC, NT, NT, W, W, prec, st))) return rc;
-    S2_TRACE("final_layer -> FC", w.FC, (size_t)NT * W * esz);
-    if ((rc = s2_gemm(h, w.FC, W, h->w_c2, h->b_c2, d_out, C, NT, C, W, EPI_STORE_F32, st))) return rc;
+    const void* fl = dedup ? (const void*)w.BIG : (const void*)w.FC;
+    S2_TRACE("final_layer -> FC", fl, (size_t)NT * W * esz);
+    if ((rc = s2_gemm(h, fl, W, h->w_c2, h->b_c2, d_out, C, NT, C, W, EPI_STORE_F32, st))) return rc;
     S2_TRACE("conv2 -> output", d_out, (size_t)NT * C * 4);
     return ITTS_OK;
 #undef S2_TRACE
diff --git a/indextts_amd/csrc/common.h b/indextts_amd/csrc/common.h
--- a/indextts_amd/csrc/common.h
+++ b/indextts_amd/csrc/common.h
@@ -23,7 +23,8 @@
 
 enum { OPT_DECODE_FUSE_LN, OPT_DECODE_GEMM, OPT_DECODE_ROT, OPT_DECODE_WNT, OPT_DECODE_NT, OPT_PREFILL_GEMM, OPT_TILE256, OPT_F32_TILE,
        OPT_X3_PRODUCTS, OPT_X3_SCHED, OPT_X3_ATTN, OPT_SAMPLE_RADIX, OPT_GPT_COMPACT, OPT_ATTN_WAVES, OPT_S2MEL_FUSED, OPT_FA_QS,
-       OPT_F32_ATTN_SCALAR, OPT_FA32_QS, OPT_AA_ACT, OPT_CONV_BM, OPT_H3_KERNEL, OPT_DECODE_LN_NT, OPT_X3_APLANES, OPT_X3_PIN, OPT_PREFILL_ATTN, OPT_VOC_ACT_PLANES, OPT_X3_WAVES, OPT_S2MEL_PRUNE_LAST, OPT_X3_ATTN_SKIP, OPT_COUNT };
+       OPT_F32_ATTN_SCALAR, OPT_FA32_QS, OPT_AA_ACT, OPT_CONV_BM, OPT_H3_KERNEL, OPT_DECODE_LN_NT, OPT_X3_APLANES, OPT_X3_PIN, OPT_PREFILL_ATTN, OPT_VOC_ACT_PLANES, OPT_X3_WAVES, OPT_S2MEL_PRUNE_LAST, OPT_X3_ATTN_SKIP,
+       OPT_S2MEL_DEDUP, OPT_S2MEL_SKIP_FUSE, OPT_COUNT };
 int itts_opt(int id);
 unsigned itts_opt_epoch();
 
diff --git a/indextts_amd/csrc/gemm_tile.h b/indextts_amd/csrc/gemm_tile.h
--- a/indextts_amd/csrc/gemm_tile.h
+++ b/indextts_amd/csrc/gemm_tile.h
@@ -365,5 +365,6 @@
     return (a.N % 4 == 0) && (a.ldo % 4 == 0 || (a.epi != EPI_STORE_F32 && a.epi != EPI_RESIDUAL && a.epi != EPI_RESIDUAL_SRC && a.epi != EPI_GELU_ACT)) && (a.D % 4 == 0);
 }
 static inline bool pf_f32_ok(const GemmArgs& a) {
+    if (a.A2 && !(a.Wp2 && a.k_split > 0 && a.k_split < a.K && a.k_split % 32 == 0 && a.lda2 % 4 == 0 && (((uintptr_t)a.A2) & 15) == 0)) return false;
     return a.K % 32 == 0 && a.lda % 4 == 0 && a.nsplit == 1 && a.epi != EPI_PARTIAL && pf_vec_ok(a) && (((uintptr_t)a.A) & 15) == 0;
 }
diff --git a/indextts_amd/csrc/gemm_x3.hip b/indextts_amd/csrc/gemm_x3.hip
--- a/indextts_amd/csrc/gemm_x3.hip
+++ b/indextts_amd/csrc/gemm_x3.hip
@@ -23,7 +23,7 @@
     }
 }
 
-template <int EPI, bool CONV = false, int NPROD = 8, bool SCHED = true, bool APL = false>
+template <int EPI, bool CONV = false, int NPROD = 8, bool SCHED = true, bool APL = false, bool SRC2 = false>
 __global__ __launch_bounds__(256, 2) void gemm_x3_kernel(GemmArgs a) {
     extern __shared__ __attribute__((aligned(16))) char pf_sm[];
     const int lane = threadIdx.x & 63, w = __builtin_amdgcn_readfirstlane(threadIdx.x >> 6);
@@ -44,6 +44,10 @@
     const char* asrc[APL ? 6 : 4];
     uint32_t aoff[APL ? 6 : 4];
     const char* abase = (const char*)a.A + (size_t)m0 * a.lda * (APL ? 2 : 4);
+    static_assert(!SRC2 || (!APL && !CONV), "two sources: f32 row operands only");
+    const int ks = SRC2 ? a.k_split >> 5 : nk;
+    const char* abase2 = SRC2 ? (const char*)a.A2 + (size_t)m0 * a.lda2 * 4 : nullptr;
+    uint32_t arow[SRC2 ? 4 : 1], apiece[SRC2 ? 4 : 1];
     int cv_t[4], cv_T[4];
     const char* cv_base[4];
     const char* cv_zero[4];
@@ -69,6 +73,7 @@
         m = m < a.M ? m : a.M - 1;
         asrc[i] = (const char*)a.A + (size_t)m * a.lda * 4 + piece * 16;
         aoff[i] = (uint32_t)(m - m0) * (uint32_t)a.lda * 4u + piece * 16;
+        if constexpr (SRC2) { arow[i] = (uint32_t)(m - m0); apiece[i] = piece * 16; }
         if constexpr (CONV) {
             const int sq = a.tok_seq[m];
             cv_t[i] = a.tok_t[m];
@@ -79,12 +84,14 @@
     }
     }
     const char* wbase[4];
+    const char* wbase2[SRC2 ? 4 : 1];
     const uint32_t lane16 = lane * 16;
 #pragma unroll
     for (int nt = 0; nt < 4; ++nt) {
         int ntile = nt0 + wc * 4 + nt;
         ntile = ntile < ntiles ? ntile : ntiles - 1;
-        wbase[nt] = (const char*)a.Wp + (size_t)ntile * nk * 3072;
+        wbase[nt] = (const char*)a.Wp + (size_t)ntile * ks * 3072;
+        if constexpr (SRC2) wbase2[nt] = (const char*)a.Wp2 + (size_t)ntile * (nk - ks) * 3072;
     }
     auto issue_a = [&](int kt, int buf) {
         char* base = pf_sm + buf * STAGE;
@@ -112,7 +119,13 @@
             if constexpr (CONV)
                 __builtin_amdgcn_global_load_lds((const __attribute__((address_space(1))) void*)ap,
                                                  (__attribute__((address_space(3))) void*)(base + (w * 4 + i) * 1024), 16, 0, 0);
-            else
+            else if constexpr (SRC2) {
+                const bool sec = kt >= ks;
+                const char* ab = sec ? abase2 + (size_t)(kt - ks) * 128 : abase + (size_t)kt * 128;
+                const uint32_t ld4 = (uint32_t)(sec ? a.lda2 : a.lda) * 4u;
+                __builtin_amdgcn_global_load_lds((const __attribute__((address_space(1))) void*)(pf_uni(ab) + (__umul24(arow[i], ld4) + apiece[i])),
+                                                 (__attribute__((address_space(3))) void*)(base + (w * 4 + i) * 1024), 16, 0, 0);
+            } else
                 __builtin_amdgcn_global_load_lds((const __attribute__((address_space(1))) void*)(pf_uni(abase + (size_t)kt * 128) + aoff[i]),
                                                  (__attribute__((address_space(3))) void*)(base + (w * 4 + i) * 1024), 16, 0, 0);
         }
@@ -121,7 +134,11 @@
 #pragma unroll
         for (int nt = 0; nt < 4; ++nt)
 #pragma unroll
-            for (int p = 0; p < 3; ++p) bw[nt][p] = *(const __attribute__((address_space(1))) v4u*)(pf_uni(wbase[nt] + (size_t)kt * 3072) + lane16 + p * 1024);
+            for (int p = 0; p < 3; ++p) {
+                const char* wb = wbase[nt] + (size_t)kt * 3072;
+                if constexpr (SRC2) { if (kt >= ks) wb = wbase2[nt] + (size_t)(kt - ks) * 3072; }
+                bw[nt][p] = *(const __attribute__((address_space(1))) v4u*)(pf_uni(wb) + lane16 + p * 1024);
+            }
     };
 
     f32x4 acc[4][4];
@@ -227,7 +244,7 @@
 
 #define X3W8_STAGE (16384 + 24576)
 #define X3W8_LDS (2 * X3W8_STAGE)
-template <int EPI, bool CONV = false>
+template <int EPI, bool CONV = false, bool SRC2 = false>
 __global__ __launch_bounds__(512, 2) void gemm_x3w8_kernel(GemmArgs a) {
     extern __shared__ __attribute__((aligned(16))) char pf_sm[];
     constexpr int NPROD = 6;
@@ -248,6 +265,10 @@
     const char* asrc[2];
     uint32_t aoff[2];
     const char* abase = (const char*)a.A + (size_t)m0 * a.lda * 4;
+    static_assert(!SRC2 || !CONV, "two sources: f32 row operands only");
+    const int ks = SRC2 ? a.k_split >> 5 : nk;
+    const char* abase2 = SRC2 ? (const char*)a.A2 + (size_t)m0 * a.lda2 * 4 : nullptr;
+    uint32_t arow[SRC2 ? 2 : 1], apiece[SRC2 ? 2 : 1];
     int cv_t[2], cv_T[2];
     const char* cv_base[2];
     const char* cv_zero[2];
@@ -262,6 +283,7 @@
         m = m < a.M ? m : a.M - 1;
         asrc[i] = (const char*)a.A + (size_t)m * a.lda * 4 + piece * 16;
         aoff[i] = (uint32_t)(m - m0) * (uint32_t)a.lda * 4u + piece * 16;
+        if constexpr (SRC2) { arow[i] = (uint32_t)(m - m0); apiece[i] = piece * 16; }
         if constexpr (CONV) {
             const int sq = a.tok_seq[m];
             cv_t[i] = a.tok_t[m];
@@ -271,13 +293,15 @@
         }
     }
     const char* wdma[3];
+    const char* wdma2[SRC2 ? 3 : 1];
     const uint32_t lane16 = lane * 16;
 #pragma unroll
     for (int i = 0; i < 3; ++i) {
         const int q = w + 8 * i;
         int ntile = nt0 + q / 3;
         ntile = ntile < ntiles ? ntile : ntiles - 1;
-        wdma[i] = (const char*)a.Wp + (size_t)ntile * nk * 3072 + (q % 3) * 1024;
+        wdma[i] = (const char*)a.Wp + (size_t)ntile * ks * 3072 + (q % 3) * 1024;
+        if constexpr (SRC2) wdma2[i] = (const char*)a.Wp2 + (size_t)ntile * (nk - ks) * 3072 + (q % 3) * 1024;
     }
     auto issue = [&](int kt, int buf) {
         char* base = pf_sm + buf * X3W8_STAGE;
@@ -295,6 +319,13 @@
                 const char* ap = ok ? cv_base[i] + ((size_t)p * a.lda + (size_t)rem * 32) * 4 : cv_zero[i];
                 __builtin_amdgcn_global_load_lds((const __attribute__((address_space(1))) void*)ap,
                                                  (__attribute__((address_space(3))) void*)(base + (w * 2 + i) * 1024), 16, 0, 0);
+            } else if constexpr (SRC2) {
+                (void)asrc;
+                const bool sec = kt >= ks;
+                const char* ab = sec ? abase2 + (size_t)(kt - ks) * 128 : abase + (size_t)kt * 128;
+                const uint32_t ld4 = (uint32_t)(sec ? a.lda2 : a.lda) * 4u;
+                __builtin_amdgcn_global_load_lds((const __attribute__((address_space(1))) void*)(pf_uni(ab) + (__umul24(arow[i], ld4) + apiece[i])),
+                                                 (__attribute__((address_space(3))) void*)(base + (w * 2 + i) * 1024), 16, 0, 0);
             } else {
                 (void)asrc;
                 __builtin_amdgcn_global_load_lds((const __attribute__((address_space(1))) void*)(pf_uni(abase + (size_t)kt * 128) + aoff[i]),
@@ -302,9 +333,12 @@
             }
         }
 #pragma unroll
-        for (int i = 0; i < 3; ++i)
-            __builtin_amdgcn_global_load_lds((const __attribute__((address_space(1))) void*)(pf_uni(wdma[i] + (size_t)kt * 3072) + lane16),
+        for (int i = 0; i < 3; ++i) {
+            const char* wb = wdma[i] + (size_t)kt * 3072;
+            if constexpr (SRC2) { if (kt >= ks) wb = wdma2[i] + (size_t)(kt - ks) * 3072; }
+            __builtin_amdgcn_global_load_lds((const __attribute__((address_space(1))) void*)(pf_uni(wb) + lane16),
                                              (__attribute__((address_space(3))) void*)(base + 16384 + (w + 8 * i) * 1024), 16, 0, 0);
+        }
     };
 
     f32x4 acc[2][4];
@@ -422,6 +456,36 @@
             return ITTS_OK;
         }
     } else if (a.a_planes) { itts_set_error("gemm (f32x3): plane operands are supported for the wqkv / SwiGLU GEMMs only"); return ITTS_ERR_ARG; }
+    if constexpr (!CONV && EPI == EPI_STORE_F32) {
+        if (a.A2) {
+            if (a.a_planes || a.lda < a.k_split || a.lda2 < a.K - a.k_split || a.lda >= (1 << 22) || a.lda2 >= (1 << 22)) {
+                itts_set_error("gemm (f32x3): two sources need f32 rows with k_split <= lda < 2^22 and K - k_split <= lda2 < 2^22");
+                return ITTS_ERR_ARG;
+            }
+            static ItPerDevice<bool> s2_set_pd;
+            bool& s2_set = s2_set_pd.cur();
+            if (!s2_set) {
+                HIP_TRY(hipFuncSetAttribute((const void*)gemm_x3_kernel<EPI, CONV, 8, true, false, true>, hipFuncAttributeMaxDynamicSharedMemorySize, X3_LDS_ONE));
+                HIP_TRY(hipFuncSetAttribute((const void*)gemm_x3_kernel<EPI, CONV, 6, true, false, true>, hipFuncAttributeMaxDynamicSharedMemorySize, X3_LDS_ONE));
+                HIP_TRY(hipFuncSetAttribute((const void*)gemm_x3_kernel<EPI, CONV, 8, false, false, true>, hipFuncAttributeMaxDynamicSharedMemorySize, X3_LDS_ONE));
+                HIP_TRY(hipFuncSetAttribute((const void*)gemm_x3_kernel<EPI, CONV, 6, false, false, true>, hipFuncAttributeMaxDynamicSharedMemorySize, X3_LDS_ONE));
+                HIP_TRY(hipFuncSetAttribute((const void*)gemm_x3w8_kernel<EPI, CONV, true>, hipFuncAttributeMaxDynamicSharedMemorySize, X3W8_LDS));
+                s2_set = true;
+            }
+            if (nprod == 6 && sched && itts_opt(OPT_X3_WAVES) == 8 && itts_opt(OPT_X3_PIN) == 0) {
+                gemm_note_path(GP_X3_8W);
+                hipLaunchKernelGGL((gemm_x3w8_kernel<EPI, CONV, true>), grid, dim3(512), X3W8_LDS, st, a);
+            } else {
+                gemm_note_path(nprod == 6 ? GP_X3_4W_P6 : GP_X3_4W_P8);
+                if (nprod == 6 && sched) hipLaunchKernelGGL((gemm_x3_kernel<EPI, CONV, 6, true, false, true>), grid, blk, lds, st, a);
+                else if (nprod == 6) hipLaunchKernelGGL((gemm_x3_kernel<EPI, CONV, 6, false, false, true>), grid, blk, lds, st, a);
+                else if (sched) hipLaunchKernelGGL((gemm_x3_kernel<EPI, CONV, 8, true, false, true>), grid, blk, lds, st, a);
+                else hipLaunchKernelGGL((gemm_x3_kernel<EPI, CONV, 8, false, false, true>), grid, blk, lds, st, a);
+            }
+            HIP_TRY(hipGetLastError());
+            return ITTS_OK;
+        }
+    } else if (a.A2) { itts_set_error("gemm (f32x3): a second A source is supported for the plain f32 store epilogue only (no tap mode, no plane operands)"); return ITTS_ERR_ARG; }
     if (nprod == 6 && sched && itts_opt(OPT_X3_WAVES) == 8 && itts_opt(OPT_X3_PIN) == 0) {
         static ItPerDevice<bool> w8_set_pd;
         bool& w8_set = w8_set_pd.cur();
@@ -445,8 +509,8 @@
 
 int launch_gemm_x3(const GemmArgs& a, hipStream_t st) {
     if (!pf_f32_ok(a)) {
-        itts_set_error("gemm (f32x3): needs K %% 32 == 0, lda %% 4 == 0, N / ldo / D %% 4 == 0, 16-byte aligned rows, no split-K (M=%d N=%d K=%d lda=%d epi=%d)",
-                       a.M, a.N, a.K, a.lda, a.epi);
+        itts_set_error("gemm (f32x3): needs K %% 32 == 0, lda %% 4 == 0, N / ldo / D %% 4 == 0, 16-byte aligned rows, no split-K; a second source needs Wp2, 0 < k_split < K, "
+                       "k_split %% 32 == 0, lda2 %% 4 == 0 (M=%d N=%d K=%d lda=%d epi=%d k_split=%d lda2=%d)", a.M, a.N, a.K, a.lda, a.epi, a.k_split, a.lda2);
         return ITTS_ERR_ARG;
     }
     if (a.epi == EPI_GATE && a.conv_taps > 0 &&
diff --git a/indextts_amd/csrc/gpt_kernels.h b/indextts_amd/csrc/gpt_kernels.h
--- a/indextts_amd/csrc/gpt_kernels.h
+++ b/indextts_amd/csrc/gpt_kernels.h
@@ -52,6 +52,7 @@
     size_t kv_planes;
     const float* res_src;
     const int* res_map;
+    const void* A2; int lda2; const void* Wp2; int k_split;
 };
 int launch_gemm(const GemmArgs& a, int prec, bool prefill, hipStream_t st);
 int launch_gemm_x3(const GemmArgs& a, hipStream_t st);
diff --git a/indextts_amd/csrc/gpt_kernels.hip b/indextts_amd/csrc/gpt_kernels.hip
--- a/indextts_amd/csrc/gpt_kernels.hip
+++ b/indextts_amd/csrc/gpt_kernels.hip
@@ -1641,6 +1641,7 @@
         return ITTS_ERR_ARG;
     }
     if (a.nsplit > 1 && a.epi != EPI_PARTIAL) { itts_set_error("gemm: split-K needs EPI_PARTIAL"); return ITTS_ERR_ARG; }
+    if (a.A2 && prec != PREC_F32X3) { itts_set_error("gemm: a second A source (A2) exists for the fp32x3 tile kernel only"); return ITTS_ERR_ARG; }
     if (prec == PREC_F32X3) return launch_gemm_x3(a, st);
     return prec == PREC_BF16 ? launch_gemm_t<true>(a, prefill, st) : launch_gemm_t<false>(a, prefill, st);
 }
diff --git a/indextts_amd/csrc/options.hip b/indextts_amd/csrc/options.hip
--- a/indextts_amd/csrc/options.hip
+++ b/indextts_amd/csrc/options.hip
@@ -42,6 +42,8 @@
     {"x3_waves", 8, 4, 8, "fp32x3 GEMM: waves per 128 x 128 block -- 8 (4 x 2, wave tile 32 x 64, weights through LDS: four waves per SIMD at two blocks per CU; 64-utterance solve 314.7 vs 323.0 ms per Euler step, profiles/r06k) or 4 (2 x 2, wave tile 64 x 64, weights in registers: round 5's kernel); bitwise equal", "4,8"},
     {"s2mel_prune_last", 1, 0, 1, "fp32x3 s2mel solve with a tail layout: the LAST DiT layer's attention runs the queries of the tail rows only (keys / values: every frame) and writes the tail layout, its wo / FFN norm / w1|w3 / w2 stages run on the tail rows (residual gathered by a row map in the wo epilogue); the x_in GEMM reads its residual from const_in instead of a copy of it; 0: every row, copy first (bitwise equal)"},
     {"x3_attn_skip", 1, 0, 1, "fp32x3 flash attention: a last key tile with <= 32 valid keys skips the MFMAs of its fully masked half, and a wave whose 32 queries are all out of range only stages its share of K / V^T (0: full tiles, every wave computes; bitwise equal)"},
+    {"s2mel_dedup", 1, 0, 1, "fp32x3 s2mel: no second f32 copy of a matrix the same epilogue has just written (the bf16 mode's operand shadows are bit-for-bit duplicates when the activation element is f32) -- the saved U-ViT skip IS the stream buffer (w2 out of place into SK[i], the next wo out of place back), skip_in / conv1 / res_projection / the tap-mode in_layer / conv2 read the f32 output itself, and the workspace drops WXA; 0: the shadow stores (bitwise equal)"},
+    {"s2mel_skip_fuse", 1, 0, 1, "fp32x3 s2mel: skip_in_linear([x | skip]) and skip_linear([norm(x) | x^T]) as ONE two-source GEMM each (K tiles of the first operand, then of the second, into one accumulator) instead of a store launch + a read-add-store launch; 0: the two launches (their low bits differ: one accumulation chain instead of (acc_a + b) + acc_b)"},
 };
 std::atomic<int> g_val[OPT_COUNT];
 std::atomic<unsigned> g_epoch{1};
diff --git a/indextts_amd/gpt.py b/indextts_amd/gpt.py
--- a/indextts_amd/gpt.py
+++ b/indextts_amd/gpt.py
@@ -1424,6 +1424,21 @@
         return out
 
 
+def gemm_cat(a: torch.Tensor, w_packed: torch.Tensor, a2: torch.Tensor, w2_packed: torch.Tensor, bias: Optional[torch.Tensor], N: int,
+             precision: int = 2) -> torch.Tensor:
+    M, K1 = a.shape
+    K2 = a2.shape[1]
+    a = a.contiguous()
+    if a2.stride(1) != 1:
+        a2 = a2.contiguous()
+    out = torch.empty(M, N, dtype=torch.float32, device=a.device)
+    with _lib.on_device(a.device):
+        _lib.check(_lib.lib().itts_gemm_cat_forward(_lib.ptr(a), K1, _lib.ptr(w_packed), _lib.ptr(a2), a2.stride(0), _lib.ptr(w2_packed), _lib.ptr(bias),
+                                                    _lib.ptr(out), M, N, K1, K2, precision, _lib.stream_ptr(a.device)),
+                   "itts_gemm_cat_forward")
+        return out
+
+
 def linear_f32(x: torch.Tensor, weight: torch.Tensor, bias: Optional[torch.Tensor], cache: Optional[dict] = None, key=None) -> torch.Tensor:
     N, K = weight.shape
     if K % 16:
```

After: 142.7, median of 6. Within noise of the previous version (+0.5%).
